# antoine311200/sow

Hardware: AMD Instinct MI355X
Metric: SoWLinear fwd+bwd tokens/s, llama_60m rank=50 (56-layer SoWLinear stack) (higher is better)
Workload: dtype bf16

## Files before the change

sow_amd/csrc/api.hip:

```cpp
#include "kernels.hpp"
#include <cstring>
#include <vector>
#include <cstdio>
#include <cstdlib>

namespace sow {

template <typename T, typename TO>
__global__ __launch_bounds__(256) void colsum_kernel(const T* M, int64_t ld, int64_t rows, int D, TO* out, float beta) {
  __shared__ float red[4][64];
  const int c = blockIdx.x * 64 + (threadIdx.x & 63), w = threadIdx.x >> 6;
  float s = 0.f;
  if (c < D)
    for (int64_t i = w; i < rows; i += 4) s += to_f32(M[i * ld + c]);
  red[w][threadIdx.x & 63] = s;
  __syncthreads();
  if (w == 0 && c < D) {
    float v = red[0][threadIdx.x] + red[1][threadIdx.x] + red[2][threadIdx.x] + red[3][threadIdx.x];
    if (beta != 0.f) v += beta * to_f32(out[c]);
    out[c] = from_f32<TO>(v);
  }
}
static int launch_colsum(const void* dy, int64_t T, int d_out, void* dbias, float beta, int dtype, int out_dtype,
                         hipStream_t stream) {
  const dim3 grid((d_out + 63) / 64);
  if (out_dtype != dtype && out_dtype != SOW_F32) return SOW_ERR_DTYPE;
  const bool o32 = out_dtype == SOW_F32;
  if (dtype == SOW_F32)
    hipLaunchKernelGGL((colsum_kernel<float, float>), grid, dim3(256), 0, stream, (const float*)dy, (int64_t)d_out, T, d_out, (float*)dbias, beta);
  else if (dtype == SOW_BF16 && o32)
    hipLaunchKernelGGL((colsum_kernel<bf16_t, float>), grid, dim3(256), 0, stream, (const bf16_t*)dy, (int64_t)d_out, T, d_out, (float*)dbias, beta);
  else if (dtype == SOW_BF16)
    hipLaunchKernelGGL((colsum_kernel<bf16_t, bf16_t>), grid, dim3(256), 0, stream, (const bf16_t*)dy, (int64_t)d_out, T, d_out, (bf16_t*)dbias, beta);
  else if (dtype == SOW_F16 && o32)
    hipLaunchKernelGGL((colsum_kernel<f16_t, float>), grid, dim3(256), 0, stream, (const f16_t*)dy, (int64_t)d_out, T, d_out, (float*)dbias, beta);
  else if (dtype == SOW_F16)
    hipLaunchKernelGGL((colsum_kernel<f16_t, f16_t>), grid, dim3(256), 0, stream, (const f16_t*)dy, (int64_t)d_out, T, d_out, (f16_t*)dbias, beta);
  else
    return SOW_ERR_DTYPE;
  SOW_CHECK_LAUNCH();
  return SOW_OK;
}
}

namespace sow {
static const char* const kSwitchNames[SW_COUNT] = {"FORCE_CHAIN_V1", "NO_SHORT_SPLIT", "NO_FUSED_H", "FORCE_GEMM_V1", "TN_NARROW",
                                                   "NO_GEMM3S",      "GEMM3S",         "GEMM3",      "NO_GROUPED",     "NO_PERSIST",     "NO_NT_STORE",    "NT_LOAD",        "NO_PAIR_FLUSH",  "F32_EXACT",
                                                   "NO_PARK16",      "TN_NO_NT_LOAD",  "NO_TN_ROWS",     "GEMM4",          "NO_GEMM4H",      "NO_CHAIN3F",     "NO_TN_F32Q",     "NO_SPLITK",
                                                   "NO_WIDE_CHAIN",  "NO_SHARED_X",    "NO_RAGGED",      "NO_RAGGED_GEMM", "NO_BLOCKED_QR",
                                                   "NO_SKINNY"};
static std::atomic<int> g_switch[SW_COUNT];
static std::once_flag g_switch_once;
static void switches_from_env() {
  for (int i = 0; i < SW_COUNT; ++i) {
    char name[64];
    snprintf(name, sizeof name, "SOW_AMD_%s", kSwitchNames[i]);
    const char* v = getenv(name);
    const bool tri = i == SW_GEMM3S || i == SW_GEMM3 || i == SW_GEMM4;
    g_switch[i].store(!v ? -1 : (tri ? (v[0] != '0') : 1), std::memory_order_relaxed);
  }
}
int sw(int which) {
  std::call_once(g_switch_once, switches_from_env);
  return g_switch[which].load(std::memory_order_relaxed);
}
}

using namespace sow;

static inline size_t al256(size_t v) { return (v + 255) & ~(size_t)255; }
static inline size_t esize(int dtype) { return dtype == SOW_F32 ? 4 : 2; }
static inline bool ok_dtype(int d) { return d == SOW_F32 || d == SOW_BF16 || d == SOW_F16; }
static inline bool al4p(const void* p) { return (reinterpret_cast<uintptr_t>(p) & 3) == 0; }
static inline bool al16p(const void* p) { return (reinterpret_cast<uintptr_t>(p) & 15) == 0; }
static inline int split_dtype(int d, bool* pf) {
  *pf = (d & SOW_PARAM_F32) != 0;
  const int cd = d & ~SOW_PARAM_F32;
  if (!ok_dtype(cd) || (*pf && cd == SOW_F32)) return -1;
  return cd;
}
static inline bool flagged(int d) { return (d & SOW_PARAM_F32) != 0; }

constexpr int SHORT_NTB = 128;
static inline int short_want(int ntb) { return ntb > 0 ? (256 + ntb - 1) / ntb : 1; }
static size_t short_hp_bytes(int64_t T, int d_in, int d_out, int r_live, int dtype) {
  const int ntb = ceil_div(T, 64);
  if (r_live > 64 || ntb <= 0 || ntb > SHORT_NTB) return 0;
  const int dmax = d_in > d_out ? d_in : d_out;
  int ks = short_want(ntb);
  const int nst = (dmax + 63) / 64;
  if (ks > nst) ks = nst;
  return al256((size_t)ks * (size_t)T * 64 * sizeof(float));
}
static int launch_chain_short(const ChainParams& p, int dtype, bool bwd, float* hpartial, hipStream_t stream) {
  const int ntb = ceil_div(p.M, 64);
  const bool f32 = dtype == SOW_F32;
  if (!hpartial || !p.Hsave || ntb > SHORT_NTB || !(f32 ? chain2f_supported(p, dtype) : chain2_supported(p, dtype)) ||
      sw_on(SW_FORCE_CHAIN_V1) || sw_on(SW_NO_SHORT_SPLIT))
    return SOW_ERR_UNSUPPORTED;
  const int want = short_want(ntb);
  const int nst = (p.D1 + 63) / 64, nsl = (p.D2 + 63) / 64;
  if (nst + nsl < 24) return SOW_ERR_UNSUPPORTED;
  int rc;
  int ks = want < nst ? want : nst;
  if (ks > 1) {
    ChainParams a = p;
    a.ntb = ntb, a.st_per = ceil_div(nst, ks), a.sl_per = 0, a.Hpartial = hpartial, a.Hload = nullptr;
    ks = ceil_div(nst, a.st_per);
    rc = f32 ? launch_chain2f(a, bwd, stream) : launch_chain2(a, bwd, dtype, stream);
    if (rc) return rc == SOW_ERR_ALIGN ? SOW_ERR_UNSUPPORTED : rc;
    rc = launch_h_reduce(hpartial, ks, p.Hsave, p.M, p.rb, p.scale, dtype, stream);
    if (rc) return rc;
  } else {
    ChainParams a = p;
    a.Y = nullptr, a.D2 = 0, a.bias = nullptr;
    rc = f32 ? launch_chain2f(a, bwd, stream) : launch_chain2(a, bwd, dtype, stream);
    if (rc) return rc == SOW_ERR_ALIGN ? SOW_ERR_UNSUPPORTED : rc;
  }
  if (nsl == 0) return SOW_OK;
  ChainParams b = p;
  const int kn = want < nsl ? want : nsl;
  b.ntb = ntb, b.st_per = 0, b.sl_per = ceil_div(nsl, kn), b.Hpartial = nullptr, b.Hload = p.Hsave, b.Hsave = nullptr;
  return f32 ? launch_chain2f(b, bwd, stream) : launch_chain2(b, bwd, dtype, stream);
}

static int gemm_auto(const void* A, int64_t lda, const void* B, int64_t ldb, bool transB, void* C, int64_t ldc,
                     const void* bias, int64_t M, int N, int K, float alpha, float beta, int dtype, hipStream_t stream,
                     void* ws = nullptr, size_t ws_bytes = 0) {
  if (dtype == SOW_F16) {
    const int g4 = sw(SW_GEMM4);
    const int64_t work = (int64_t)ceil_div(M, 256) * ceil_div(N, 256) * gemm4_splits(M, N, K, false, ws, ws_bytes);
    if (!sw_on(SW_FORCE_GEMM_V1) && (g4 > 0 || (g4 < 0 && work >= 120)) &&
        gemm4_supported(A, lda, B, ldb, transB, nullptr, 0, nullptr, 0, C, ldc, bias, M, N, K, dtype))
      return launch_gemm4(A, lda, B, ldb, transB, nullptr, 0, nullptr, 0, 0, C, ldc, bias, M, N, K, alpha, beta, stream, ws,
                          ws_bytes, dtype);
    return launch_gemm(A, lda, false, B, ldb, transB, C, ldc, bias, M, N, K, alpha, beta, dtype, stream);
  }
  if (gemm2_supported(A, lda, B, ldb, transB, nullptr, 0, nullptr, 0, C, ldc, bias, M, N, K, dtype))
    return launch_gemm2(A, lda, B, ldb, transB, nullptr, 0, nullptr, 0, 0, C, ldc, bias, M, N, K, alpha, beta, stream, ws, ws_bytes);
  return launch_gemm(A, lda, false, B, ldb, transB, C, ldc, bias, M, N, K, alpha, beta, dtype, stream);
}

extern "C" {

int sow_version(void) { return 118; }

int sow_set_switch(const char* name, int value) {
  if (!name) return SOW_ERR_NULL;
  (void)sw(0);
  for (int i = 0; i < SW_COUNT; ++i)
    if (!strcmp(name, kSwitchNames[i])) {
      g_switch[i].store(value < 0 ? -1 : (value != 0), std::memory_order_relaxed);
      return SOW_OK;
    }
  return SOW_ERR_UNSUPPORTED;
}

#ifdef SOW_STAMPS
int sow_debug_set_stamps(void* buf) {
  g_chain2_stamps = buf;
  return SOW_OK;
}
#endif

int sow_get_switch(const char* name) {
  if (!name) return SOW_ERR_NULL;
  for (int i = 0; i < SW_COUNT; ++i)
    if (!strcmp(name, kSwitchNames[i])) return sw(i);
  return SOW_ERR_UNSUPPORTED;
}

const char* sow_error_string(int code) {
  switch (code) {
    case SOW_OK: return "ok";
    case SOW_ERR_NULL: return "null pointer argument";
    case SOW_ERR_SHAPE: return "invalid shape argument";
    case SOW_ERR_DTYPE: return "unsupported dtype";
    case SOW_ERR_ALIGN: return "misaligned pointer";
    case SOW_ERR_WORKSPACE: return "workspace too small";
    case SOW_ERR_UNSUPPORTED: return "unsupported configuration";
    default: return code > 0 ? hipGetErrorString((hipError_t)code) : "unknown error";
  }
}

size_t sow_h_save_elems(int64_t T, int r_live) { return (size_t)T * (size_t)(r_live <= 64 ? 64 : r_live); }

static bool rag_layer(int r_live, int r_acc, int acc_kind, int d_in, int d_out, int dtype) {
  return r_live > 64 && ragged_shape_ok(r_live, d_in, d_out, dtype) &&
         (acc_kind == SOW_ACC_NONE || acc_kind == SOW_ACC_DENSE ||
          (acc_kind == SOW_ACC_LOWRANK && ragged_shape_ok(r_acc, d_in, d_out, dtype)));
}

static int rag_dense_product(const void* A, int64_t lda, const void* B, int64_t ldb, bool transB, void* C, int64_t ldc, int64_t M,
                             int N, int K, int dtype, hipStream_t stream) {
  if (!sw_on(SW_NO_RAGGED_GEMM) && gemm_rag_supported(A, lda, B, ldb, transB, C, ldc, M, N, K, dtype))
    return launch_gemm_rag(A, lda, B, ldb, transB, C, ldc, M, N, K, dtype, stream);
  return gemm_auto(A, lda, B, ldb, transB, C, ldc, nullptr, M, N, K, 1.f, 0.f, dtype, stream);
}

struct WsPlan {
  size_t off_dh, off_t, off_apad, off_hp, off_p0, off_p1, off_planes, planes_bytes, off_sk, sk_bytes, off_wide, wide_bytes,
      off_pw, pw_bytes, total;
  int ns, slab_len;
  int ns_cap;
};
constexpr int64_t C3F_MIN_T = 8192;
static WsPlan plan_ws(int64_t T, int d_in, int d_out, int r_live, int r_acc, int acc_kind, int dtype) {
  WsPlan w{};
  const size_t es = esize(dtype);
  size_t off = 0;
  w.off_dh = off;
  off += al256((size_t)T * (size_t)(r_live <= 64 ? 64 : r_live) * es);
  w.off_t = off;
  if (acc_kind == SOW_ACC_LOWRANK && r_acc > 64) off += al256((size_t)T * r_acc * es);
  w.off_apad = off;
  if (acc_kind == SOW_ACC_DENSE && r_live <= 64) off += al256((size_t)d_in * 64 * es);
  w.off_hp = off;
  off += short_hp_bytes(T, d_in, d_out, r_live, dtype);
  if (r_live <= 64) {
    const int cg_in = (d_in + 63) / 64, cg_out = (d_out + 63) / 64;
    const int quads = (dtype == SOW_F32 && tn_f32q_shape_ok(T, d_in, d_out)) ? (cg_in + 3) / 4 + (cg_out + 3) / 4 : 0;
    w.ns = tn_pick_slabs(T, cg_in + cg_out, (cg_in + 1) / 2 + (cg_out + 1) / 2, quads, dtype, &w.slab_len);
    w.ns_cap = w.ns;
    if (dtype == SOW_BF16 && T >= 1024) {
      const int by_len = (int)(T / 512 < TNR_MAX_SLABS ? T / 512 : TNR_MAX_SLABS);
      if (by_len > w.ns_cap) w.ns_cap = by_len;
    }
    w.off_p0 = off;
    off += al256(tn_partial_bytes(w.ns_cap, d_in));
    w.off_p1 = off;
    off += al256(tn_partial_bytes(w.ns_cap, d_out));
  }
  w.off_planes = off;
  w.planes_bytes = 0;
  if (dtype == SOW_F32 && T >= C3F_MIN_T && (r_live <= 64 || (acc_kind == SOW_ACC_LOWRANK && r_acc <= 64))) {
    w.planes_bytes = chain3f_plane_bytes(d_in, d_out);
    off += al256(w.planes_bytes);
  }
  w.off_sk = off;
  w.sk_bytes = 0;
  if (dtype == SOW_BF16 && acc_kind == SOW_ACC_DENSE) {
    const size_t f = gemm4_splitk_bytes(T, d_out, d_in, true), b = gemm4_splitk_bytes(T, d_in, d_out, true);
    w.sk_bytes = f > b ? f : b;
    off += al256(w.sk_bytes);
  }
  w.off_wide = off;
  w.wide_bytes = 0;
  {
    int rw = chain_wide_shape_ok(r_live, d_in, d_out, dtype) ? r_live : 0;
    if (acc_kind == SOW_ACC_LOWRANK && chain_wide_shape_ok(r_acc, d_in, d_out, dtype) && r_acc > rw) rw = r_acc;
    if (rag_layer(r_live, r_acc, acc_kind, d_in, d_out, dtype)) rw = acc_kind == SOW_ACC_LOWRANK && r_acc > r_live ? r_acc : r_live;
    if (rw) {
      w.wide_bytes = chain_wide_pack_bytes(rw, d_in, d_out);
      off += al256(w.wide_bytes);
    }
  }
  w.off_pw = off;
  w.pw_bytes = 0;
  if (tnw_shape_ok(r_live, d_in, d_out, dtype) || rag_layer(r_live, r_acc, acc_kind, d_in, d_out, dtype)) {
    w.pw_bytes = tnw_partial_bytes(T, d_in, d_out, r_live);
    off += al256(w.pw_bytes);
  }
  w.total = off;
  return w;
}

static char* ws_base(void* workspace) {
  uintptr_t a = reinterpret_cast<uintptr_t>(workspace);
  return reinterpret_cast<char*>((a + 255) & ~(uintptr_t)255);
}
static void set_planes(ChainParams& p, char* ws, const WsPlan& w, size_t workspace_bytes) {
  if (ws && w.planes_bytes && workspace_bytes >= w.total) p.planes = ws + w.off_planes, p.planes_bytes = w.planes_bytes;
}

static inline size_t pack_elems_bytes(int64_t n) { return al256((size_t)n * 2); }
static size_t pack_bytes(int d_in, int d_out, int r_live, int r_acc, int acc_kind) {
  size_t b = pack_elems_bytes((int64_t)d_in * r_live) + pack_elems_bytes((int64_t)r_live * d_out) + pack_elems_bytes(d_out);
  if (acc_kind == SOW_ACC_DENSE) b += pack_elems_bytes((int64_t)d_in * d_out);
  if (acc_kind == SOW_ACC_LOWRANK) b += pack_elems_bytes((int64_t)d_in * r_acc) + pack_elems_bytes((int64_t)r_acc * d_out);
  return b;
}
static int pack_layer(sow_layer_args& L, int cd, bool fwd, std::vector<PackItem>& items) {
  const int r_acc = L.acc_kind == SOW_ACC_LOWRANK ? L.r_acc : 0;
  const WsPlan w = plan_ws(L.T, L.d_in, L.d_out, L.r_live, r_acc, L.acc_kind, cd);
  const size_t pack = pack_bytes(L.d_in, L.d_out, L.r_live, r_acc, L.acc_kind);
  const bool no_scratch = fwd && sow_forward_workspace_bytes(L.T, L.d_in, L.d_out, L.r_live, r_acc, L.acc_kind, cd) == 0;
  const size_t off = (no_scratch && L.workspace_bytes < w.total + pack + 255) ? 0 : w.total;
  if (!L.workspace) return SOW_ERR_NULL;
  if (L.workspace_bytes < off + pack + 255) return SOW_ERR_WORKSPACE;
  char* dst = ws_base(L.workspace) + off;
  if (no_scratch) L.workspace = nullptr, L.workspace_bytes = 0;
  auto put = [&](const void*& src, int64_t n) {
    if (!src) return;
    items.push_back(PackItem{(const float*)src, dst, n});
    src = dst;
    dst += pack_elems_bytes(n);
  };
  put(L.A, (int64_t)L.d_in * L.r_live);
  put(L.B, (int64_t)L.r_live * L.d_out);
  put(L.bias, L.d_out);
  if (L.acc_kind == SOW_ACC_DENSE) put(L.acc_down, (int64_t)L.d_in * L.d_out);
  if (L.acc_kind == SOW_ACC_LOWRANK) {
    put(L.acc_down, (int64_t)L.d_in * r_acc);
    put(L.acc_up, (int64_t)r_acc * L.d_out);
  }
  return SOW_OK;
}
static sow_layer_args single_layer(const void* A, const void* B, const void* acc_down, const void* acc_up, const void* bias,
                                   int64_t T, int d_in, int d_out, int r_live, int r_acc, int acc_kind, void* workspace,
                                   size_t workspace_bytes) {
  sow_layer_args L{};
  L.A = A, L.B = B, L.acc_down = acc_down, L.acc_up = acc_up, L.bias = bias;
  L.T = T, L.d_in = d_in, L.d_out = d_out, L.r_live = r_live, L.r_acc = r_acc, L.acc_kind = acc_kind;
  L.workspace = workspace, L.workspace_bytes = workspace_bytes;
  return L;
}

static int wide_chain(const void* X, void* Y, const void* F1, int64_t ldf1, const void* F2, int64_t ldf2, void* Hsave,
                      const void* bias, int64_t T, int D1, int D2, int r, float hscale, float yscale, float beta, bool bwd,
                      int dtype, char* ws, const WsPlan& w, size_t workspace_bytes, hipStream_t stream, bool rag = false) {
  const bool ragged = D1 % 8 != 0 || D2 % 8 != 0;
  if ((ragged ? !rag : sw_on(SW_NO_WIDE_CHAIN)) || !ws || !w.wide_bytes || workspace_bytes < w.total + 255 ||
      chain_wide_pack_bytes(r, D1, D2) > w.wide_bytes)
    return SOW_ERR_UNSUPPORTED;
  WideArgs a{};
  a.X = X, a.Y = Y, a.F1 = F1, a.F2 = F2, a.ldf1 = ldf1, a.ldf2 = ldf2, a.Hsave = Hsave, a.bias = bias;
  a.M = T, a.D1 = D1, a.D2 = D2, a.r = r, a.hscale = hscale, a.yscale = yscale, a.beta = beta, a.bwd = bwd ? 1 : 0;
  a.pack = ws + w.off_wide, a.pack_bytes = w.wide_bytes;
  return launch_chain_wide(a, dtype, stream);
}

static ReduceParams make_reduce_params(const WsPlan& w, char* ws, void* dA, void* dB, void* dbias_ones, int d_in, int d_out,
                                       int r_live, float grad_beta) {
  ReduceParams rp{};
  rp.njobs = 2, rp.ns = w.ns;
  rp.job[0] = ReduceJob{(const float*)(ws + w.off_p0), dA, nullptr, (int64_t)r_live, d_in, (d_in + 63) / 64 * 64, r_live, 0, -1,
                        1.f, grad_beta};
  rp.job[1] = ReduceJob{(const float*)(ws + w.off_p1), dB, dbias_ones, (int64_t)d_out, d_out, (d_out + 63) / 64 * 64, r_live, 1,
                        dbias_ones ? 63 : -1, 1.f , grad_beta};
  rp.blocks0 = (d_in + 3) / 4;
  return rp;
}

size_t sow_reduce_desc_bytes(void) { return sizeof(ReduceParams); }

int sow_backward_reduce_desc(void* dA, void* dB, void* dbias, int64_t T, int d_in, int d_out, int r_live, int r_acc,
                             int acc_kind, float grad_beta, int dtype, void* workspace, size_t workspace_bytes, void* desc_out,
                             int* blocks_out) {
  bool pf;
  dtype = split_dtype(dtype, &pf);
  if (dtype < 0) return SOW_ERR_DTYPE;
  if (T <= 0 || d_in <= 0 || d_out <= 0 || r_live <= 0) return SOW_ERR_SHAPE;
  if (!dA || !dB || !workspace || !desc_out || !blocks_out) return SOW_ERR_NULL;
  if (r_live > 64) {
    memset(desc_out, 0, sizeof(ReduceParams));
    *blocks_out = 0;
    return SOW_OK;
  }
  if (dbias && r_live > 63) return SOW_ERR_UNSUPPORTED;
  if (acc_kind != SOW_ACC_LOWRANK) r_acc = 0;
  const WsPlan w = plan_ws(T, d_in, d_out, r_live, r_acc, acc_kind, dtype);
  if (workspace_bytes < w.total + 255) return SOW_ERR_WORKSPACE;
  const ReduceParams rp = make_reduce_params(w, ws_base(workspace), dA, dB, dbias, d_in, d_out, r_live, grad_beta);
  memcpy(desc_out, &rp, sizeof(rp));
  *blocks_out = (d_in + 3) / 4 + (d_out + 3) / 4;
  return SOW_OK;
}

int sow_reduce_batch(const void* descs, const int* starts, int n, int total_blocks, int dtype, void* stream) {
  bool pf;
  const int cd = split_dtype(dtype, &pf);
  if (cd < 0) return SOW_ERR_DTYPE;
  if (pf) dtype = SOW_F32;
  if (n < 0 || total_blocks < 0) return SOW_ERR_SHAPE;
  if (n == 0) return SOW_OK;
  if (!descs || !starts) return SOW_ERR_NULL;
  return launch_tn_reduce_batch((const ReduceParams*)descs, starts, n, total_blocks, dtype, (hipStream_t)stream);
}

size_t sow_forward_workspace_bytes(int64_t T, int d_in, int d_out, int r_live, int r_acc, int acc_kind, int dtype) {
  bool pf;
  dtype = split_dtype(dtype, &pf);
  if (T < 0 || d_in <= 0 || d_out <= 0 || r_live <= 0 || dtype < 0) return 0;
  if (pf) {
    const size_t own = sow_forward_workspace_bytes(T, d_in, d_out, r_live, r_acc, acc_kind, dtype);
    const size_t pack = pack_bytes(d_in, d_out, r_live, acc_kind == SOW_ACC_LOWRANK ? r_acc : 0, acc_kind);
    return own ? own + pack : pack + 256;
  }
  const bool wide_acc = acc_kind == SOW_ACC_LOWRANK && r_acc > 64;
  const WsPlan w = plan_ws(T, d_in, d_out, r_live, r_acc, acc_kind, dtype);
  if (!wide_acc && r_live <= 64 && short_hp_bytes(T, d_in, d_out, r_live, dtype) == 0 && w.planes_bytes == 0 && w.sk_bytes == 0)
    return 0;
  return w.total + 256;
}

size_t sow_workspace_bytes(int64_t T, int d_in, int d_out, int r_live, int r_acc, int acc_kind, int dtype) {
  bool pf;
  dtype = split_dtype(dtype, &pf);
  if (T < 0 || d_in <= 0 || d_out <= 0 || r_live <= 0 || dtype < 0) return 0;
  const size_t pack = pf ? pack_bytes(d_in, d_out, r_live, acc_kind == SOW_ACC_LOWRANK ? r_acc : 0, acc_kind) : 0;
  return plan_ws(T, d_in, d_out, r_live, r_acc, acc_kind, dtype).total + pack + 256;
}


static int forward_impl(const void* x, const void* A, const void* B, const void* acc_down, const void* acc_up, const void* bias,
                        void* y, void* h_save, int64_t T, int d_in, int d_out, int r_live, int r_acc, int acc_kind, float scale,
                        int dtype, void* workspace, size_t workspace_bytes, void* stream_) {
  hipStream_t stream = (hipStream_t)stream_;
  if (!ok_dtype(dtype)) return SOW_ERR_DTYPE;
  if (T < 0 || d_in <= 0 || d_out <= 0 || r_live <= 0) return SOW_ERR_SHAPE;
  if (T == 0) return SOW_OK;
  if (!x || !A || !B || !y) return SOW_ERR_NULL;
  if (acc_kind != SOW_ACC_NONE && !acc_down) return SOW_ERR_NULL;
  if (acc_kind == SOW_ACC_LOWRANK && (!acc_up || r_acc <= 0)) return SOW_ERR_SHAPE;
  if (acc_kind != SOW_ACC_LOWRANK) r_acc = 0;
  const WsPlan w = plan_ws(T, d_in, d_out, r_live, r_acc, acc_kind, dtype);
  char* ws = workspace ? ws_base(workspace) : nullptr;
  float beta = 0.f;
  int rc;
  if (rag_layer(r_live, r_acc, acc_kind, d_in, d_out, dtype) && !sw_on(SW_NO_RAGGED) && ws && workspace_bytes >= w.total + 255 &&
      al16p(x) && al16p(y) && (!bias || al16p(bias)) && (!h_save || al4p(h_save))) {
    if (acc_kind == SOW_ACC_LOWRANK) {
      rc = wide_chain(x, y, acc_down, r_acc, acc_up, d_out, nullptr, nullptr, T, d_in, d_out, r_acc, 1.f, 1.f, 0.f, false, dtype,
                      ws, w, workspace_bytes, stream, true);
      if (rc) return rc;
      beta = 1.f;
    } else if (acc_kind == SOW_ACC_DENSE) {
      rc = rag_dense_product(x, d_in, acc_down, d_out, false, y, d_out, T, d_out, d_in, dtype, stream);
      if (rc) return rc;
      beta = 1.f;
    }
    return wide_chain(x, y, A, r_live, B, d_out, h_save, bias, T, d_in, d_out, r_live, 1.f, scale, beta, false, dtype, ws, w,
                      workspace_bytes, stream, true);
  }
  if (acc_kind == SOW_ACC_DENSE) {
    if (r_live <= 64 && h_save) {
      if (gemm4h_supported(x, d_in, acc_down, d_out, false, A, r_live, B, d_out, y, d_out, bias, h_save, T, d_out, d_in, r_live,
                           dtype))
        return launch_gemm4h(x, d_in, acc_down, d_out, false, A, r_live, B, d_out, y, d_out, bias, h_save, T, d_out, d_in,
                             r_live, scale, dtype, stream);
      if (gemm2h_supported(x, d_in, acc_down, d_out, false, A, r_live, B, d_out, y, d_out, bias, h_save, T, d_out, d_in,
                           r_live, dtype))
        return launch_gemm2h(x, d_in, acc_down, d_out, false, A, r_live, B, d_out, y, d_out, bias, h_save, T, d_out, d_in,
                             r_live, scale, stream);
      ChainParams ph{};
      ph.X = x, ph.Y = nullptr, ph.Hsave = h_save, ph.bias = nullptr;
      ph.M = T, ph.ldx = d_in, ph.ldy = d_out, ph.D1 = d_in, ph.D2 = 0;
      ph.F1b = A, ph.ldf1b = r_live, ph.F2b = B, ph.ldf2b = d_out, ph.rb = r_live;
      ph.scale = scale, ph.beta = 0.f;
      set_planes(ph, ws, w, workspace_bytes);
      if (chain2_supported(ph, dtype) &&
          gemm2_supported(x, d_in, acc_down, d_out, false, h_save, 64, B, d_out, y, d_out, bias, T, d_out, d_in, dtype)) {
        rc = SOW_ERR_UNSUPPORTED;
        if (ws && workspace_bytes >= w.total) rc = launch_chain_short(ph, dtype, false, (float*)(ws + w.off_hp), stream);
        if (rc == SOW_ERR_UNSUPPORTED) rc = launch_chain2(ph, false, dtype, stream);
        if (rc) return rc;
        const bool sk = ws && w.sk_bytes && workspace_bytes >= w.total;
        return launch_gemm2(x, d_in, acc_down, d_out, false, h_save, 64, B, d_out, r_live, y, d_out, bias, T, d_out, d_in,
                            1.f, 0.f, stream, sk ? ws + w.off_sk : nullptr, sk ? w.sk_bytes : 0);
      }
    }
    rc = gemm_auto(x, d_in, acc_down, d_out, false, y, d_out, nullptr, T, d_out, d_in, 1.f, 0.f, dtype, stream);
    if (rc) return rc;
    beta = 1.f;
  } else if (acc_kind == SOW_ACC_LOWRANK) {
    if (r_acc <= 64) {
      ChainParams p{};
      p.X = x, p.Y = y, p.Hsave = nullptr, p.bias = nullptr;
      p.M = T, p.ldx = d_in, p.ldy = d_out, p.D1 = d_in, p.D2 = d_out;
      p.F1b = acc_down, p.ldf1b = r_acc, p.F2b = acc_up, p.ldf2b = d_out, p.rb = r_acc;
      p.scale = 1.f, p.beta = 0.f;
      set_planes(p, ws, w, workspace_bytes);
      rc = launch_chain(p, dtype, false, stream);
      if (rc) return rc;
      beta = 1.f;
    } else {
      if (!ws || workspace_bytes < w.total) return SOW_ERR_WORKSPACE;
      rc = wide_chain(x, y, acc_down, r_acc, acc_up, d_out, nullptr, nullptr, T, d_in, d_out, r_acc, 1.f, 1.f, 0.f, false, dtype,
                      ws, w, workspace_bytes, stream);
      if (rc == SOW_ERR_UNSUPPORTED) {
        void* t = ws + w.off_t;
        rc = launch_gemm(x, d_in, false, acc_down, r_acc, false, t, r_acc, nullptr, T, r_acc, d_in, 1.f, 0.f, dtype, stream);
        if (rc) return rc;
        rc = launch_gemm(t, r_acc, false, acc_up, d_out, false, y, d_out, nullptr, T, d_out, r_acc, 1.f, 0.f, dtype, stream);
      }
      if (rc) return rc;
      beta = 1.f;
    }
  }
  if (r_live <= 64) {
    ChainParams p{};
    p.X = x, p.Y = y, p.Hsave = h_save, p.bias = bias;
    p.M = T, p.ldx = d_in, p.ldy = d_out, p.D1 = d_in, p.D2 = d_out;
    p.F1b = A, p.ldf1b = r_live, p.F2b = B, p.ldf2b = d_out, p.rb = r_live;
    p.scale = scale, p.beta = beta;
    set_planes(p, ws, w, workspace_bytes);
    if (ws && workspace_bytes >= w.total) {
      rc = launch_chain_short(p, dtype, false, (float*)(ws + w.off_hp), stream);
      if (rc != SOW_ERR_UNSUPPORTED) return rc;
    }
    return launch_chain(p, dtype, false, stream);
  }
  const bool ws_ok = ws && workspace_bytes >= w.total + 255;
  rc = wide_chain(x, y, A, r_live, B, d_out, h_save, bias, T, d_in, d_out, r_live, 1.f, scale, beta, false, dtype, ws, w,
                  workspace_bytes, stream);
  if (rc != SOW_ERR_UNSUPPORTED) return rc;
  void* h = h_save;
  if (!h) {
    if (!ws_ok) return SOW_ERR_WORKSPACE;
    h = ws + w.off_dh;
  }
  rc = launch_gemm(x, d_in, false, A, r_live, false, h, r_live, nullptr, T, r_live, d_in, 1.f, 0.f, dtype, stream);
  if (rc) return rc;
  return launch_gemm(h, r_live, false, B, d_out, false, y, d_out, bias, T, d_out, r_live, scale, beta, dtype, stream);
}

int sow_forward(const void* x, const void* A, const void* B, const void* acc_down, const void* acc_up, const void* bias,
                void* y, void* h_save, int64_t T, int d_in, int d_out, int r_live, int r_acc, int acc_kind, float scale,
                int dtype, void* workspace, size_t workspace_bytes, void* stream) {
  bool pf;
  const int cd = split_dtype(dtype, &pf);
  if (cd < 0) return SOW_ERR_DTYPE;
  if (!pf)
    return forward_impl(x, A, B, acc_down, acc_up, bias, y, h_save, T, d_in, d_out, r_live, r_acc, acc_kind, scale, dtype,
                        workspace, workspace_bytes, stream);
  if (T < 0 || d_in <= 0 || d_out <= 0 || r_live <= 0) return SOW_ERR_SHAPE;
  if (T == 0) return SOW_OK;
  if (!x || !A || !B || !y) return SOW_ERR_NULL;
  if (acc_kind != SOW_ACC_NONE && !acc_down) return SOW_ERR_NULL;
  if (acc_kind == SOW_ACC_LOWRANK && (!acc_up || r_acc <= 0)) return SOW_ERR_SHAPE;
  if (acc_kind != SOW_ACC_LOWRANK) r_acc = 0, acc_up = nullptr;
  if (acc_kind == SOW_ACC_NONE) acc_down = nullptr;
  sow_layer_args L = single_layer(A, B, acc_down, acc_up, bias, T, d_in, d_out, r_live, r_acc, acc_kind, workspace, workspace_bytes);
  std::vector<PackItem> items;
  int rc = pack_layer(L, cd, true, items);
  if (rc) return rc;
  if ((rc = launch_pack_params(items.data(), (int)items.size(), cd, (hipStream_t)stream))) return rc;
  return forward_impl(x, L.A, L.B, L.acc_down, L.acc_up, L.bias, y, h_save, T, d_in, d_out, r_live, r_acc, acc_kind, scale, cd,
                      L.workspace, L.workspace_bytes, stream);
}

static int backward_impl(const void* dy, const void* x, const void* h_save, const void* A, const void* B, const void* acc_down,
                         const void* acc_up, void* dx, void* dA, void* dB, void* dbias, int64_t T, int d_in, int d_out,
                         int r_live, int r_acc, int acc_kind, float scale, float grad_beta, int dtype, int gdt, void* workspace,
                         size_t workspace_bytes, int phases, void* stream_) {
  hipStream_t stream = (hipStream_t)stream_;
  bool do_data = (phases & SOW_BWD_DATA) != 0;
  const bool do_partial = (phases & (SOW_BWD_WEIGHTS | SOW_BWD_WEIGHTS_PARTIAL)) != 0;
  const bool do_reduce = (phases & (SOW_BWD_WEIGHTS | SOW_BWD_WEIGHTS_REDUCE)) != 0;
  const bool do_weights = do_partial || do_reduce;
  if (!do_data && !do_weights) return SOW_ERR_SHAPE;
  if (!ok_dtype(dtype)) return SOW_ERR_DTYPE;
  if (T < 0 || d_in <= 0 || d_out <= 0 || r_live <= 0) return SOW_ERR_SHAPE;
  if (T == 0) {
    if (!dA || !dB) return SOW_ERR_NULL;
    if (grad_beta == 0.f) {
      void* ptrs[3] = {dA, dB, dbias};
      int64_t bytes[3] = {(int64_t)d_in * r_live * (int64_t)esize(gdt), (int64_t)r_live * d_out * (int64_t)esize(gdt),
                          dbias ? (int64_t)d_out * (int64_t)esize(gdt) : 0};
      return launch_multi_zero(ptrs, bytes, 3, stream);
    }
    return SOW_OK;
  }
  if (!dy || !x || !h_save || !A || !B || !dx || !dA || !dB || !workspace) return SOW_ERR_NULL;
  if (acc_kind != SOW_ACC_NONE && !acc_down) return SOW_ERR_NULL;
  if (acc_kind == SOW_ACC_LOWRANK && (!acc_up || r_acc <= 0)) return SOW_ERR_SHAPE;
  if (acc_kind != SOW_ACC_LOWRANK) r_acc = 0;
  const WsPlan w = plan_ws(T, d_in, d_out, r_live, r_acc, acc_kind, dtype);
  if (workspace_bytes < w.total + 255) return SOW_ERR_WORKSPACE;
  char* ws = ws_base(workspace);
  void* dh = ws + w.off_dh;
  float beta = 0.f;
  int rc;
  bool data_done = false;
  const bool rag_w = rag_layer(r_live, r_acc, acc_kind, d_in, d_out, dtype) && !sw_on(SW_NO_RAGGED);
  if (rag_w && do_data && al16p(dy) && al16p(dx)) {
    if (acc_kind == SOW_ACC_LOWRANK) {
      rc = wide_chain(dy, dx, acc_up, d_out, acc_down, r_acc, nullptr, nullptr, T, d_out, d_in, r_acc, 1.f, 1.f, 0.f, true, dtype,
                      ws, w, workspace_bytes, stream, true);
      if (rc) return rc;
      beta = 1.f;
    } else if (acc_kind == SOW_ACC_DENSE) {
      rc = rag_dense_product(dy, d_out, acc_down, d_out, true, dx, d_in, T, d_in, d_out, dtype, stream);
      if (rc) return rc;
      beta = 1.f;
    }
    rc = wide_chain(dy, dx, B, d_out, A, r_live, dh, nullptr, T, d_out, d_in, r_live, scale, 1.f, beta, true, dtype, ws, w,
                    workspace_bytes, stream, true);
    if (rc) return rc;
    do_data = false;
  }
  if (!do_data) {
  } else if (acc_kind == SOW_ACC_DENSE) {
    if (r_live <= 64) {
      ChainParams pd{};
      pd.X = dy, pd.Y = nullptr, pd.Hsave = dh, pd.bias = nullptr;
      pd.M = T, pd.ldx = d_out, pd.ldy = d_in, pd.D1 = d_out, pd.D2 = 0;
      pd.F1b = B, pd.ldf1b = d_out, pd.F2b = A, pd.ldf2b = r_live, pd.rb = r_live;
      pd.scale = scale, pd.beta = 0.f;
      set_planes(pd, ws, w, workspace_bytes);
      void* apad = ws + w.off_apad;
      if (gemm4h_supported(dy, d_out, acc_down, d_out, true, B, d_out, A, r_live, dx, d_in, nullptr, dh, T, d_in, d_out, r_live,
                           dtype)) {
        rc = launch_gemm4h(dy, d_out, acc_down, d_out, true, B, d_out, A, r_live, dx, d_in, nullptr, dh, T, d_in, d_out, r_live,
                           scale, dtype, stream);
        if (rc) return rc;
        data_done = true;
      } else if (gemm2h_supported(dy, d_out, acc_down, d_out, true, B, d_out, A, r_live, dx, d_in, nullptr, dh, T, d_in, d_out,
                           r_live, dtype)) {
        rc = launch_gemm2h(dy, d_out, acc_down, d_out, true, B, d_out, A, r_live, dx, d_in, nullptr, dh, T, d_in, d_out,
                           r_live, scale, stream);
        if (rc) return rc;
        data_done = true;
      } else if (chain2_supported(pd, dtype) &&
          gemm2_supported(dy, d_out, acc_down, d_out, true, dh, 64, apad, 64, dx, d_in, nullptr, T, d_in, d_out, dtype)) {
        const bool pad_fused = (int64_t)ceil_div(T, 64) * 64 >= d_in;
        if (pad_fused) pd.pad_src = A, pd.pad_dst = apad, pd.pad_rows = d_in, pd.pad_r = r_live;
        rc = SOW_ERR_UNSUPPORTED;
        if (short_hp_bytes(T, d_in, d_out, r_live, dtype)) rc = launch_chain_short(pd, dtype, true, (float*)(ws + w.off_hp), stream);
        if (rc == SOW_ERR_UNSUPPORTED) rc = launch_chain2(pd, true, dtype, stream);
        if (rc) return rc;
        if (!pad_fused) {
          rc = launch_pad64(A, apad, d_in, r_live, stream);
          if (rc) return rc;
        }
        rc = launch_gemm2(dy, d_out, acc_down, d_out, true, dh, 64, apad, 64, 64, dx, d_in, nullptr, T, d_in, d_out, 1.f, 0.f,
                          stream, w.sk_bytes ? ws + w.off_sk : nullptr, w.sk_bytes);
        if (rc) return rc;
        data_done = true;
      }
    }
    if (!data_done) rc = gemm_auto(dy, d_out, acc_down, d_out, true, dx, d_in, nullptr, T, d_in, d_out, 1.f, 0.f, dtype, stream);
    if (rc) return rc;
    beta = 1.f;
  } else if (acc_kind == SOW_ACC_LOWRANK) {
    if (r_acc <= 64) {
      ChainParams p{};
      p.X = dy, p.Y = dx, p.Hsave = nullptr, p.bias = nullptr;
      p.M = T, p.ldx = d_out, p.ldy = d_in, p.D1 = d_out, p.D2 = d_in;
      p.F1b = acc_up, p.ldf1b = d_out, p.F2b = acc_down, p.ldf2b = r_acc, p.rb = r_acc;
      p.scale = 1.f, p.beta = 0.f;
      set_planes(p, ws, w, workspace_bytes);
      rc = launch_chain(p, dtype, true, stream);
      if (rc) return rc;
      beta = 1.f;
    } else {
      rc = wide_chain(dy, dx, acc_up, d_out, acc_down, r_acc, nullptr, nullptr, T, d_out, d_in, r_acc, 1.f, 1.f, 0.f, true, dtype,
                      ws, w, workspace_bytes, stream);
      if (rc == SOW_ERR_UNSUPPORTED) {
        void* t = ws + w.off_t;
        rc = launch_gemm(dy, d_out, false, acc_up, d_out, true, t, r_acc, nullptr, T, r_acc, d_out, 1.f, 0.f, dtype, stream);
        if (rc) return rc;
        rc = launch_gemm(t, r_acc, false, acc_down, r_acc, true, dx, d_in, nullptr, T, d_in, r_acc, 1.f, 0.f, dtype, stream);
      }
      if (rc) return rc;
      beta = 1.f;
    }
  }
  if (r_live <= 64) {
    ChainParams p{};
    p.X = dy, p.Y = dx, p.Hsave = dh, p.bias = nullptr;
    p.M = T, p.ldx = d_out, p.ldy = d_in, p.D1 = d_out, p.D2 = d_in;
    p.F1b = B, p.ldf1b = d_out, p.F2b = A, p.ldf2b = r_live, p.rb = r_live;
    p.scale = scale, p.beta = beta;
    set_planes(p, ws, w, workspace_bytes);
    if (do_data && !data_done) {
      rc = launch_chain_short(p, dtype, true, short_hp_bytes(T, d_in, d_out, r_live, dtype) ? (float*)(ws + w.off_hp) : nullptr, stream);
      if (rc == SOW_ERR_UNSUPPORTED) rc = launch_chain(p, dtype, true, stream);
      if (rc) return rc;
    }
    if (!do_weights) return SOW_OK;
    const bool ones_ok = dbias && r_live <= 63;
    TnParams tp{};
    tp.njobs = 2, tp.T = T, tp.ns = w.ns, tp.slab_len = w.slab_len;
    auto vec_ok = [&](const void* ptr, int D) {
      if (dtype == SOW_F32) return (D % 4 == 0 && al16p(ptr)) ? 1 : 0;
      return (D % 2 == 0 && al4p(ptr)) ? 1 : 0;
    };
    tp.job[0] = TnJob{x, dh, (float*)(ws + w.off_p0), (int64_t)d_in, d_in, -1, (d_in + 63) / 64, vec_ok(x, d_in), 1};
    tp.job[1] = TnJob{dy, h_save, (float*)(ws + w.off_p1), (int64_t)d_out, d_out, ones_ok ? 63 : -1, (d_out + 63) / 64,
                      vec_ok(dy, d_out), 1};
    if (do_partial) {
      rc = launch_tn(tp, dtype, stream);
      if (rc) return rc;
    }
    if (!do_reduce) return SOW_OK;
    const ReduceParams rp = make_reduce_params(w, ws, dA, dB, ones_ok ? dbias : nullptr, d_in, d_out, r_live, grad_beta);
    rc = launch_tn_reduce(rp, gdt, stream);
    if (rc) return rc;
    if (dbias && !ones_ok) {
      rc = launch_colsum(dy, T, d_out, dbias, grad_beta, dtype, gdt, stream);
      if (rc) return rc;
    }
    return SOW_OK;
  }
  if (do_data) {
    rc = wide_chain(dy, dx, B, d_out, A, r_live, dh, nullptr, T, d_out, d_in, r_live, scale, 1.f, beta, true, dtype, ws, w,
                    workspace_bytes, stream);
    if (rc == SOW_ERR_UNSUPPORTED) {
      rc = launch_gemm(dy, d_out, false, B, d_out, true, dh, r_live, nullptr, T, r_live, d_out, scale, 0.f, dtype, stream);
      if (rc) return rc;
      rc = launch_gemm(dh, r_live, false, A, r_live, true, dx, d_in, nullptr, T, d_in, r_live, 1.f, beta, dtype, stream);
    }
    if (rc) return rc;
  }
  if (!do_partial) return SOW_OK;
  if (w.pw_bytes && (rag_w || (!sw_on(SW_NO_WIDE_CHAIN) && tnw_shape_ok(r_live, d_in, d_out, dtype)))) {
    rc = launch_tn_wide(x, dh, dy, h_save, dA, dB, dbias, T, d_in, d_out, r_live, scale, grad_beta, dtype, gdt, ws + w.off_pw,
                        w.pw_bytes, stream);
    if (rc != SOW_ERR_UNSUPPORTED) return rc;
  }
  rc = launch_gemm_out(x, d_in, true, dh, r_live, false, dA, r_live, nullptr, d_in, r_live, (int)T, 1.f, grad_beta, dtype, gdt,
                       stream);
  if (rc) return rc;
  rc = launch_gemm_out(h_save, r_live, true, dy, d_out, false, dB, d_out, nullptr, r_live, d_out, (int)T, scale, grad_beta, dtype,
                       gdt, stream);
  if (rc) return rc;
  if (dbias) {
    rc = launch_colsum(dy, T, d_out, dbias, grad_beta, dtype, gdt, stream);
    if (rc) return rc;
  }
  return SOW_OK;
}

int sow_backward_ex(const void* dy, const void* x, const void* h_save, const void* A, const void* B, const void* acc_down,
                    const void* acc_up, void* dx, void* dA, void* dB, void* dbias, int64_t T, int d_in, int d_out,
                    int r_live, int r_acc, int acc_kind, float scale, float grad_beta, int dtype, void* workspace,
                    size_t workspace_bytes, int phases, void* stream) {
  bool pf;
  const int cd = split_dtype(dtype, &pf);
  if (!pf)
    return backward_impl(dy, x, h_save, A, B, acc_down, acc_up, dx, dA, dB, dbias, T, d_in, d_out, r_live, r_acc, acc_kind, scale,
                         grad_beta, dtype, dtype, workspace, workspace_bytes, phases, stream);
  if (cd < 0) return SOW_ERR_DTYPE;
  if ((phases & SOW_BWD_DATA) && T > 0) {
    if (d_in <= 0 || d_out <= 0 || r_live <= 0) return SOW_ERR_SHAPE;
    if (!dy || !x || !h_save || !A || !B || !dx || !dA || !dB || !workspace) return SOW_ERR_NULL;
    if (acc_kind != SOW_ACC_NONE && !acc_down) return SOW_ERR_NULL;
    if (acc_kind == SOW_ACC_LOWRANK && (!acc_up || r_acc <= 0)) return SOW_ERR_SHAPE;
    if (acc_kind != SOW_ACC_LOWRANK) r_acc = 0, acc_up = nullptr;
    if (acc_kind == SOW_ACC_NONE) acc_down = nullptr;
    sow_layer_args L = single_layer(A, B, acc_down, acc_up, nullptr, T, d_in, d_out, r_live, r_acc, acc_kind, workspace,
                                    workspace_bytes);
    std::vector<PackItem> items;
    int rc = pack_layer(L, cd, false, items);
    if (rc) return rc;
    if ((rc = launch_pack_params(items.data(), (int)items.size(), cd, (hipStream_t)stream))) return rc;
    A = L.A, B = L.B, acc_down = L.acc_down, acc_up = L.acc_up;
  }
  return backward_impl(dy, x, h_save, A, B, acc_down, acc_up, dx, dA, dB, dbias, T, d_in, d_out, r_live, r_acc, acc_kind, scale,
                       grad_beta, cd, SOW_F32, workspace, workspace_bytes, phases, stream);
}

int sow_backward(const void* dy, const void* x, const void* h_save, const void* A, const void* B, const void* acc_down,
                 const void* acc_up, void* dx, void* dA, void* dB, void* dbias, int64_t T, int d_in, int d_out,
                 int r_live, int r_acc, int acc_kind, float scale, float grad_beta, int dtype, void* workspace,
                 size_t workspace_bytes, void* stream) {
  return sow_backward_ex(dy, x, h_save, A, B, acc_down, acc_up, dx, dA, dB, dbias, T, d_in, d_out, r_live, r_acc, acc_kind,
                         scale, grad_beta, dtype, workspace, workspace_bytes, SOW_BWD_DATA | SOW_BWD_WEIGHTS, stream);
}

static bool group_chain_params(const sow_layer_args& L, bool bwd, int dtype, const WsPlan& w, ChainParams* out) {
  if ((dtype != SOW_BF16 && dtype != SOW_F16) || L.acc_kind != SOW_ACC_NONE || L.r_live > 64 || sw_on(SW_NO_GROUPED) || sw_on(SW_FORCE_CHAIN_V1))
    return false;
  if (ceil_div(L.T, 64) <= SHORT_NTB) return false;
  ChainParams p{};
  if (!bwd) {
    p.X = L.x, p.Y = L.y, p.Hsave = L.h_save, p.bias = L.bias;
    p.M = L.T, p.ldx = L.d_in, p.ldy = L.d_out, p.D1 = L.d_in, p.D2 = L.d_out;
    p.F1b = L.A, p.ldf1b = L.r_live, p.F2b = L.B, p.ldf2b = L.d_out, p.rb = L.r_live;
  } else {
    p.X = L.dy, p.Y = L.dx, p.Hsave = ws_base(L.workspace) + w.off_dh, p.bias = nullptr;
    p.M = L.T, p.ldx = L.d_out, p.ldy = L.d_in, p.D1 = L.d_out, p.D2 = L.d_in;
    p.F1b = L.B, p.ldf1b = L.d_out, p.F2b = L.A, p.ldf2b = L.r_live, p.rb = L.r_live;
  }
  p.scale = L.scale, p.beta = 0.f;
  if (!chain2_supported(p, dtype)) return false;
  const void* Bp = bwd ? p.F1b : p.F2b;
  const int64_t ldB = bwd ? p.ldf1b : p.ldf2b;
  const void* Ap = bwd ? p.F2b : p.F1b;
  if ((reinterpret_cast<uintptr_t>(Bp) & 15) || ldB % 8 || (reinterpret_cast<uintptr_t>(Ap) & 3)) return false;
  *out = p;
  return true;
}

static bool group_rows_plan(const sow_layer_args* layers, int n, int dtype, int* ns, int* slab_len) {
  if (dtype != SOW_BF16 || n < 1 || n > TN_MAXG) return false;
  int64_t T[TNR_MAXI];
  int D[TNR_MAXI], cap[TNR_MAXI];
  for (int i = 0; i < n; ++i) {
    const sow_layer_args& L = layers[i];
    if (L.T <= 0 || L.r_live > 64 || (L.dbias && L.r_live > 63)) return false;
    const WsPlan w = plan_ws(L.T, L.d_in, L.d_out, L.r_live, L.acc_kind == SOW_ACC_LOWRANK ? L.r_acc : 0, L.acc_kind, dtype);
    if (L.workspace_bytes < w.total + 255) return false;
    if (L.d_in % 8 || L.d_out % 8 || !al16p(L.x) || !al16p(L.dy) || !al16p(L.h_save)) return false;
    T[2 * i] = T[2 * i + 1] = L.T;
    D[2 * i] = L.d_in, D[2 * i + 1] = L.d_out;
    cap[2 * i] = cap[2 * i + 1] = w.ns_cap;
  }
  return tn_rows_plan(T, D, cap, 2 * n, ns, slab_len);
}

static int check_layer(const sow_layer_args& L, bool bwd) {
  if (L.T < 0 || L.d_in <= 0 || L.d_out <= 0 || L.r_live <= 0) return SOW_ERR_SHAPE;
  if (L.T == 0) return SOW_OK;
  if (!L.x || !L.A || !L.B) return SOW_ERR_NULL;
  if (!bwd && !L.y) return SOW_ERR_NULL;
  if (bwd && (!L.dy || !L.h_save || !L.dx || !L.dA || !L.dB || !L.workspace)) return SOW_ERR_NULL;
  if (L.acc_kind != SOW_ACC_NONE && !L.acc_down) return SOW_ERR_NULL;
  return SOW_OK;
}

static int pack_group(const sow_layer_args* layers, int n, int cd, bool bwd, std::vector<sow_layer_args>& out, void* stream) {
  out.assign(layers, layers + n);
  std::vector<PackItem> items;
  int rc;
  for (sow_layer_args& L : out) {
    if ((rc = check_layer(L, bwd))) return rc;
    if (L.T == 0) continue;
    if (L.acc_kind == SOW_ACC_LOWRANK && (!L.acc_up || L.r_acc <= 0)) return SOW_ERR_SHAPE;
    if (L.acc_kind != SOW_ACC_LOWRANK) L.acc_up = nullptr;
    if (L.acc_kind == SOW_ACC_NONE) L.acc_down = nullptr;
    if (bwd) L.bias = nullptr;
    if ((rc = pack_layer(L, cd, !bwd, items))) return rc;
  }
  return launch_pack_params(items.data(), (int)items.size(), cd, (hipStream_t)stream);
}

static int forward_group_impl(const sow_layer_args* layers, int n, int dtype, void* stream_) {
  hipStream_t stream = (hipStream_t)stream_;
  if (!ok_dtype(dtype)) return SOW_ERR_DTYPE;
  if (n < 0) return SOW_ERR_SHAPE;
  if (n == 0) return SOW_OK;
  if (!layers) return SOW_ERR_NULL;
  ChainParams batch[C2_MAXG];
  Gemm2hArgs gbatch[4];
  int nb = 0, ng = 0, rc;
  for (int i = 0; i < n; ++i) {
    const sow_layer_args& L = layers[i];
    if ((rc = check_layer(L, false))) return rc;
    if (L.T == 0) continue;
    const WsPlan w{};
    if (group_chain_params(L, false, dtype, w, &batch[nb])) {
      if (++nb == C2_MAXG) {
        if ((rc = launch_chain2_group(batch, nb, false, dtype, stream))) return rc;
        nb = 0;
      }
      continue;
    }
    if (L.acc_kind == SOW_ACC_DENSE && L.r_live <= 64 && L.h_save &&
        gemm4h_supported(L.x, L.d_in, L.acc_down, L.d_out, false, L.A, L.r_live, L.B, L.d_out, L.y, L.d_out, L.bias, L.h_save, L.T,
                         L.d_out, L.d_in, L.r_live, dtype)) {
      if ((rc = launch_gemm4h(L.x, L.d_in, L.acc_down, L.d_out, false, L.A, L.r_live, L.B, L.d_out, L.y, L.d_out, L.bias, L.h_save,
                              L.T, L.d_out, L.d_in, L.r_live, L.scale, dtype, stream)))
        return rc;
      continue;
    }
    if (L.acc_kind == SOW_ACC_DENSE && L.r_live <= 64 && L.h_save && !sw_on(SW_NO_GROUPED) &&
        gemm2h_supported(L.x, L.d_in, L.acc_down, L.d_out, false, L.A, L.r_live, L.B, L.d_out, L.y, L.d_out, L.bias, L.h_save, L.T,
                         L.d_out, L.d_in, L.r_live, dtype)) {
      gbatch[ng] = Gemm2hArgs{L.x, L.acc_down, L.A, L.B, L.y, L.bias, L.h_save, L.T, L.d_in, L.d_out, L.r_live, L.d_out, L.d_out,
                              L.d_out, L.d_in, L.r_live, L.scale};
      if (++ng == 4) {
        if ((rc = launch_gemm2h_group(gbatch, ng, false, stream))) return rc;
        ng = 0;
      }
      continue;
    }
    rc = sow_forward(L.x, L.A, L.B, L.acc_down, L.acc_up, L.bias, L.y, L.h_save, L.T, L.d_in, L.d_out, L.r_live, L.r_acc,
                     L.acc_kind, L.scale, dtype, L.workspace, L.workspace_bytes, stream_);
    if (rc) return rc;
  }
  if (ng && (rc = launch_gemm2h_group(gbatch, ng, false, stream))) return rc;
  return nb ? launch_chain2_group(batch, nb, false, dtype, stream) : SOW_OK;
}

int sow_forward_group(const sow_layer_args* layers, int n, int dtype, void* stream) {
  bool pf;
  const int cd = split_dtype(dtype, &pf);
  if (cd < 0) return SOW_ERR_DTYPE;
  if (!pf || n <= 0 || !layers) return forward_group_impl(layers, n, cd, stream);
  std::vector<sow_layer_args> packed;
  const int rc = pack_group(layers, n, cd, false, packed, stream);
  return rc ? rc : forward_group_impl(packed.data(), n, cd, stream);
}

static bool skinny_shape_ok(int64_t T, int d_in, int d_out, int r_live, int acc_kind, int dtype) {
  return (dtype == SOW_BF16 || dtype == SOW_F16) && T >= 1 && T <= 32 && d_in > 0 && d_out > 0 && r_live >= 1 && r_live <= 64 &&
         (acc_kind == SOW_ACC_DENSE || acc_kind == SOW_ACC_NONE) && d_in % 8 == 0 && d_out % 8 == 0;
}
struct SkWs {
  size_t off_py, off_ph, total;
};
static SkWs skinny_ws(int64_t T, int d_in, int d_out, int acc_kind) {
  int S, KS, ncr;
  skinny_plan(d_in, d_out, acc_kind, &S, &KS, &ncr);
  SkWs w;
  w.off_py = 0;
  w.off_ph = acc_kind == SOW_ACC_DENSE ? al256(skinny_py_bytes(T, d_out, S)) : 0;
  w.total = 256 + w.off_ph + al256(skinny_ph_bytes(T, S));
  return w;
}

size_t sow_forward_skinny_workspace_bytes(int64_t T, int d_in, int d_out, int r_live, int acc_kind, int dtype) {
  if (!skinny_shape_ok(T, d_in, d_out, r_live, acc_kind, dtype)) return 0;
  return skinny_ws(T, d_in, d_out, acc_kind).total;
}

int sow_forward_skinny(const sow_layer_args* layers, int n, int dtype, void* stream) {
  bool pf;
  const int cd = split_dtype(dtype, &pf);
  if (cd < 0 || cd == SOW_F32) return SOW_ERR_DTYPE;
  if (pf || sw_on(SW_NO_SKINNY)) return SOW_ERR_UNSUPPORTED;
  if (n < 0) return SOW_ERR_SHAPE;
  if (n == 0) return SOW_OK;
  if (!layers) return SOW_ERR_NULL;
  if (n > SK_MAXL) return SOW_ERR_UNSUPPORTED;
  SkLayer sk[SK_MAXL];
  int m = 0;
  for (int i = 0; i < n; ++i) {
    const sow_layer_args& L = layers[i];
    if (L.T < 0 || L.d_in <= 0 || L.d_out <= 0 || L.r_live <= 0) return SOW_ERR_SHAPE;
    if (L.acc_kind != SOW_ACC_NONE && L.acc_kind != SOW_ACC_LOWRANK && L.acc_kind != SOW_ACC_DENSE) return SOW_ERR_SHAPE;
    if (L.T == 0) continue;
    if (!skinny_shape_ok(L.T, L.d_in, L.d_out, L.r_live, L.acc_kind, cd)) return SOW_ERR_UNSUPPORTED;
    const bool dense = L.acc_kind == SOW_ACC_DENSE;
    if (!L.x || !L.A || !L.B || !L.y || (dense && !L.acc_down)) return SOW_ERR_NULL;
    if (!al16p(L.x) || !al16p(L.y) || !al16p(L.A) || !al16p(L.B) || !al16p(L.bias) || (dense && !al16p(L.acc_down)))
      return SOW_ERR_UNSUPPORTED;
    const SkWs w = skinny_ws(L.T, L.d_in, L.d_out, L.acc_kind);
    if (!L.workspace || L.workspace_bytes < w.total) return SOW_ERR_WORKSPACE;
    char* ws = ws_base(L.workspace);
    SkLayer& K = sk[m++];
    K = SkLayer{};
    K.x = L.x, K.W = dense ? L.acc_down : nullptr, K.A = L.A, K.B = L.B, K.bias = L.bias, K.y = L.y;
    K.Py = dense ? (float*)(ws + w.off_py) : nullptr, K.Ph = (float*)(ws + w.off_ph);
    K.T = (int)L.T, K.d_in = L.d_in, K.d_out = L.d_out, K.r = L.r_live, K.scale = L.scale;
  }
  return launch_skinny_fwd(sk, m, cd, (hipStream_t)stream);
}

static int backward_group_impl(const sow_layer_args* layers, int n, int dtype, int gdt, int phases, void* stream_) {
  hipStream_t stream = (hipStream_t)stream_;
  const bool do_data = (phases & SOW_BWD_DATA) != 0;
  const bool do_partial = (phases & (SOW_BWD_WEIGHTS | SOW_BWD_WEIGHTS_PARTIAL)) != 0;
  const bool do_reduce = (phases & (SOW_BWD_WEIGHTS | SOW_BWD_WEIGHTS_REDUCE)) != 0;
  if (!do_data && !do_partial && !do_reduce) return SOW_ERR_SHAPE;
  if (!ok_dtype(dtype)) return SOW_ERR_DTYPE;
  if (n < 0) return SOW_ERR_SHAPE;
  if (n == 0) return SOW_OK;
  if (!layers) return SOW_ERR_NULL;
  int rc;
  for (int i = 0; i < n; ++i)
    if ((rc = check_layer(layers[i], true))) return rc;
  auto single = [&](const sow_layer_args& L, int ph) {
    return backward_impl(L.dy, L.x, L.h_save, L.A, L.B, L.acc_down, L.acc_up, L.dx, L.dA, L.dB, L.dbias, L.T, L.d_in, L.d_out,
                         L.r_live, L.r_acc, L.acc_kind, L.scale, L.grad_beta, dtype, gdt, L.workspace, L.workspace_bytes, ph,
                         stream_);
  };
  auto plan = [&](const sow_layer_args& L) {
    return plan_ws(L.T, L.d_in, L.d_out, L.r_live, L.acc_kind == SOW_ACC_LOWRANK ? L.r_acc : 0, L.acc_kind, dtype);
  };
  if (do_data) {
    ChainParams batch[C2_MAXG];
    Gemm2hArgs gbatch[4];
    int nb = 0, ng = 0;
    for (int i = 0; i < n; ++i) {
      const sow_layer_args& L = layers[i];
      if (L.T == 0) {
        if ((rc = single(L, SOW_BWD_DATA | (phases & ~SOW_BWD_DATA)))) return rc;
        continue;
      }
      const WsPlan w = plan(L);
      if (L.workspace_bytes < w.total + 255) return SOW_ERR_WORKSPACE;
      void* dh = ws_base(L.workspace) + w.off_dh;
      if (group_chain_params(L, true, dtype, w, &batch[nb])) {
        if (++nb == C2_MAXG) {
          if ((rc = launch_chain2_group(batch, nb, true, dtype, stream))) return rc;
          nb = 0;
        }
      } else if (L.acc_kind == SOW_ACC_DENSE && L.r_live <= 64 &&
                 gemm4h_supported(L.dy, L.d_out, L.acc_down, L.d_out, true, L.B, L.d_out, L.A, L.r_live, L.dx, L.d_in, nullptr, dh,
                                  L.T, L.d_in, L.d_out, L.r_live, dtype)) {
        if ((rc = launch_gemm4h(L.dy, L.d_out, L.acc_down, L.d_out, true, L.B, L.d_out, L.A, L.r_live, L.dx, L.d_in, nullptr, dh,
                                L.T, L.d_in, L.d_out, L.r_live, L.scale, dtype, stream)))
          return rc;
      } else if (L.acc_kind == SOW_ACC_DENSE && L.r_live <= 64 && !sw_on(SW_NO_GROUPED) &&
                 gemm2h_supported(L.dy, L.d_out, L.acc_down, L.d_out, true, L.B, L.d_out, L.A, L.r_live, L.dx, L.d_in, nullptr, dh,
                                  L.T, L.d_in, L.d_out, L.r_live, dtype)) {
        gbatch[ng] = Gemm2hArgs{L.dy, L.acc_down, L.B, L.A, L.dx, nullptr, dh, L.T, L.d_out, L.d_out, L.d_out, L.r_live, L.d_in,
                                L.d_in, L.d_out, L.r_live, L.scale};
        if (++ng == 4) {
          if ((rc = launch_gemm2h_group(gbatch, ng, true, stream))) return rc;
          ng = 0;
        }
      } else if ((rc = single(L, SOW_BWD_DATA)))
        return rc;
    }
    if (ng && (rc = launch_gemm2h_group(gbatch, ng, true, stream))) return rc;
    if (nb && (rc = launch_chain2_group(batch, nb, true, dtype, stream))) return rc;
  }
  int rns[TNR_MAXI], rslab[TNR_MAXI];
  const bool rows = (do_partial || do_reduce) && ((phases & SOW_BWD_GROUP_SLABS) || (do_partial && do_reduce)) &&
                    group_rows_plan(layers, n, dtype, rns, rslab);
  if (do_partial && rows) {
    TnRowsItem items[TNR_MAXI];
    for (int i = 0; i < n; ++i) {
      const sow_layer_args& L = layers[i];
      const WsPlan w = plan(L);
      char* ws = ws_base(L.workspace);
      items[2 * i] = TnRowsItem{L.x, ws + w.off_dh, (float*)(ws + w.off_p0), (int64_t)L.d_in, L.T, L.d_in, 0, 0, 0, 0, rns[2 * i],
                                rslab[2 * i], 0};
      items[2 * i + 1] = TnRowsItem{L.dy, L.h_save, (float*)(ws + w.off_p1), (int64_t)L.d_out, L.T, L.d_out, 0, 0, 0, 0,
                                    rns[2 * i + 1], rslab[2 * i + 1], 0};
    }
    if ((rc = launch_tn_rows(items, 2 * n, stream))) return rc;
  } else if (do_partial) {
    TnParams batch[TN_MAXG];
    int nb = 0;
    for (int i = 0; i < n; ++i) {
      const sow_layer_args& L = layers[i];
      if (L.T == 0) {
        if (!do_data && (rc = single(L, phases))) return rc;
        continue;
      }
      const WsPlan w = plan(L);
      if (L.workspace_bytes < w.total + 255) return SOW_ERR_WORKSPACE;
      bool grouped = false;
      if (L.r_live <= 64 && !sw_on(SW_NO_GROUPED)) {
        char* ws = ws_base(L.workspace);
        TnParams tp{};
        tp.njobs = 2, tp.T = L.T, tp.ns = w.ns, tp.slab_len = w.slab_len;
        const bool ones_ok = L.dbias && L.r_live <= 63;
        const int vx = (L.d_in % 2 == 0 && al4p(L.x)) ? 1 : 0, vy = (L.d_out % 2 == 0 && al4p(L.dy)) ? 1 : 0;
        tp.job[0] = TnJob{L.x, ws + w.off_dh, (float*)(ws + w.off_p0), (int64_t)L.d_in, L.d_in, -1, (L.d_in + 63) / 64, vx, 1};
        tp.job[1] = TnJob{L.dy, L.h_save, (float*)(ws + w.off_p1), (int64_t)L.d_out, L.d_out, ones_ok ? 63 : -1,
                          (L.d_out + 63) / 64, vy, 1};
        if (tn_group_supported(tp, dtype)) {
          batch[nb] = tp;
          grouped = true;
          if (++nb == TN_MAXG) {
            if ((rc = launch_tn_group(batch, nb, stream))) return rc;
            nb = 0;
          }
        }
      }
      if (!grouped && (rc = single(L, SOW_BWD_WEIGHTS_PARTIAL))) return rc;
    }
    if (nb && (rc = launch_tn_group(batch, nb, stream))) return rc;
  }
  if (do_reduce && rows) {
    for (int i = 0; i < n; ++i) {
      const sow_layer_args& L = layers[i];
      ReduceParams rp = make_reduce_params(plan(L), ws_base(L.workspace), L.dA, L.dB, L.dbias, L.d_in, L.d_out, L.r_live, L.grad_beta);
      rp.job[0].ns = rns[2 * i], rp.job[1].ns = rns[2 * i + 1];
      if ((rc = launch_tn_reduce(rp, gdt, stream))) return rc;
    }
  } else if (do_reduce) {
    for (int i = 0; i < n; ++i)
      if (layers[i].T != 0 && (rc = single(layers[i], SOW_BWD_WEIGHTS_REDUCE))) return rc;
  }
  return SOW_OK;
}

int sow_backward_group(const sow_layer_args* layers, int n, int dtype, int phases, void* stream) {
  bool pf;
  const int cd = split_dtype(dtype, &pf);
  if (!pf) return backward_group_impl(layers, n, dtype, dtype, phases, stream);
  if (cd < 0) return SOW_ERR_DTYPE;
  if (n <= 0 || !layers || !(phases & SOW_BWD_DATA)) return backward_group_impl(layers, n, cd, SOW_F32, phases, stream);
  std::vector<sow_layer_args> packed;
  const int rc = pack_group(layers, n, cd, true, packed, stream);
  return rc ? rc : backward_group_impl(packed.data(), n, cd, SOW_F32, phases, stream);
}

static int shared_common(const sow_layer_args* layers, int n, bool bwd) {
  if (n <= 0) return SOW_ERR_SHAPE;
  if (!layers) return SOW_ERR_NULL;
  for (int i = 0; i < n; ++i) {
    const sow_layer_args& L = layers[i];
    if (L.x != layers[0].x || L.T != layers[0].T || L.d_in != layers[0].d_in) return SOW_ERR_SHAPE;
    if (bwd && L.dx && L.dx != layers[0].dx) return SOW_ERR_SHAPE;
  }
  return SOW_OK;
}
static void shared_fill_dx(const sow_layer_args* layers, int n, sow_layer_args* out) {
  for (int i = 0; i < n; ++i) out[i] = layers[i], out[i].dx = layers[0].dx;
}

int sow_forward_shared(const sow_layer_args* layers, int n, int dtype, void* stream) {
  if (!ok_dtype(dtype & ~SOW_PARAM_F32)) return SOW_ERR_DTYPE;
  int rc;
  if ((rc = shared_common(layers, n, false))) return rc;
  for (int i = 0; i < n; ++i)
    if ((rc = check_layer(layers[i], false))) return rc;
  if (sw_on(SW_NO_SHARED_X) || flagged(dtype) || n > C2_MAXG || layers[0].T == 0) return SOW_ERR_UNSUPPORTED;
  ChainParams ps[C2_MAXG];
  for (int i = 0; i < n; ++i)
    if (!group_chain_params(layers[i], false, dtype, WsPlan{}, &ps[i])) return SOW_ERR_UNSUPPORTED;
  return launch_chain2_shared(ps, n, false, dtype, (hipStream_t)stream);
}

int sow_backward_shared(const sow_layer_args* layers, int n, int dtype, int phases, void* stream) {
  if (!ok_dtype(dtype & ~SOW_PARAM_F32)) return SOW_ERR_DTYPE;
  int rc;
  if ((rc = shared_common(layers, n, true))) return rc;
  if (n > C2_MAXG) return SOW_ERR_UNSUPPORTED;
  if (flagged(dtype)) return SOW_ERR_UNSUPPORTED;
  sow_layer_args filled[C2_MAXG];
  shared_fill_dx(layers, n, filled);
  if (!(phases & SOW_BWD_DATA)) return sow_backward_group(filled, n, dtype, phases, stream);
  for (int i = 0; i < n; ++i)
    if ((rc = check_layer(filled[i], true))) return rc;
  if (sw_on(SW_NO_SHARED_X) || filled[0].T == 0) return SOW_ERR_UNSUPPORTED;
  ChainParams ps[C2_MAXG];
  for (int i = 0; i < n; ++i) {
    const sow_layer_args& L = filled[i];
    const WsPlan w = plan_ws(L.T, L.d_in, L.d_out, L.r_live, 0, L.acc_kind, dtype);
    if (!group_chain_params(L, true, dtype, w, &ps[i])) return SOW_ERR_UNSUPPORTED;
    if (L.workspace_bytes < w.total + 255) return SOW_ERR_WORKSPACE;
    ps[i].beta = filled[0].grad_beta;
  }
  if ((rc = launch_chain2_shared(ps, n, true, dtype, (hipStream_t)stream))) return rc;
  const int wph = phases & ~SOW_BWD_DATA;
  return (wph & (SOW_BWD_WEIGHTS | SOW_BWD_WEIGHTS_PARTIAL | SOW_BWD_WEIGHTS_REDUCE))
             ? backward_group_impl(filled, n, dtype, dtype, wph, stream)
             : SOW_OK;
}

int sow_backward_group_plan(const sow_layer_args* layers, int n, int dtype, int phases, int* slabs_out) {
  bool pf;
  dtype = split_dtype(dtype, &pf);
  if (dtype < 0) return SOW_ERR_DTYPE;
  if (n < 0) return SOW_ERR_SHAPE;
  if (n == 0) return 0;
  if (!layers) return SOW_ERR_NULL;
  int rc;
  for (int i = 0; i < n; ++i)
    if ((rc = check_layer(layers[i], true))) return rc;
  const bool do_partial = (phases & (SOW_BWD_WEIGHTS | SOW_BWD_WEIGHTS_PARTIAL)) != 0;
  const bool do_reduce = (phases & (SOW_BWD_WEIGHTS | SOW_BWD_WEIGHTS_REDUCE)) != 0;
  int rns[TNR_MAXI], rslab[TNR_MAXI];
  const bool rows = (do_partial || do_reduce) && ((phases & SOW_BWD_GROUP_SLABS) || (do_partial && do_reduce)) &&
                    group_rows_plan(layers, n, dtype, rns, rslab);
  if (slabs_out)
    for (int i = 0; i < n; ++i) {
      const sow_layer_args& L = layers[i];
      int ns = 0;
      if (L.T > 0 && L.r_live <= 64)
        ns = plan_ws(L.T, L.d_in, L.d_out, L.r_live, L.acc_kind == SOW_ACC_LOWRANK ? L.r_acc : 0, L.acc_kind, dtype).ns;
      slabs_out[2 * i] = rows ? rns[2 * i] : ns;
      slabs_out[2 * i + 1] = rows ? rns[2 * i + 1] : ns;
    }
  return rows ? 1 : 0;
}

int sow_backward_group_reduce_desc(const sow_layer_args* layers, int n, int dtype, int phases, void* descs_out, int* blocks_out) {
  bool pf;
  dtype = split_dtype(dtype, &pf);
  if (dtype < 0) return SOW_ERR_DTYPE;
  if (n < 0) return SOW_ERR_SHAPE;
  if (n == 0) return SOW_OK;
  if (!layers || !descs_out || !blocks_out) return SOW_ERR_NULL;
  int rc;
  for (int i = 0; i < n; ++i)
    if ((rc = check_layer(layers[i], true))) return rc;
  int rns[TNR_MAXI], rslab[TNR_MAXI];
  const bool rows = (phases & SOW_BWD_GROUP_SLABS) && group_rows_plan(layers, n, dtype, rns, rslab);
  for (int i = 0; i < n; ++i) {
    const sow_layer_args& L = layers[i];
    char* out = (char*)descs_out + (size_t)i * sizeof(ReduceParams);
    if ((rc = sow_backward_reduce_desc(L.dA, L.dB, L.dbias, L.T, L.d_in, L.d_out, L.r_live, L.r_acc, L.acc_kind, L.grad_beta, dtype,
                                       L.workspace, L.workspace_bytes, out, blocks_out + i)))
      return rc;
    if (rows) {
      ReduceParams rp;
      memcpy(&rp, out, sizeof rp);
      rp.job[0].ns = rns[2 * i], rp.job[1].ns = rns[2 * i + 1];
      memcpy(out, &rp, sizeof rp);
    }
  }
  return SOW_OK;
}

int sow_gemm(const void* A, int64_t lda, int trans_a, const void* B, int64_t ldb, int trans_b, void* C, int64_t ldc,
             const void* bias, int64_t M, int N, int K, float alpha, float beta, int dtype, void* stream) {
  return sow_gemm_ex(A, lda, trans_a, B, ldb, trans_b, C, ldc, bias, M, N, K, alpha, beta, dtype, nullptr, 0, stream);
}

size_t sow_gemm_workspace_bytes(int64_t M, int N, int K, int trans_a, int dtype) {
  if (trans_a || (dtype != SOW_BF16 && dtype != SOW_F16) || M <= 0 || N <= 0 || K <= 0) return 0;
  return gemm4_splitk_bytes(M, N, K, false);
}

int sow_gemm_ex(const void* A, int64_t lda, int trans_a, const void* B, int64_t ldb, int trans_b, void* C, int64_t ldc,
                const void* bias, int64_t M, int N, int K, float alpha, float beta, int dtype, void* workspace,
                size_t workspace_bytes, void* stream) {
  if (flagged(dtype)) return SOW_ERR_DTYPE;
  if (!trans_a)
    return gemm_auto(A, lda, B, ldb, trans_b != 0, C, ldc, bias, M, N, K, alpha, beta, dtype, (hipStream_t)stream, workspace,
                     workspace_bytes);
  return launch_gemm(A, lda, trans_a != 0, B, ldb, trans_b != 0, C, ldc, bias, M, N, K, alpha, beta, dtype, (hipStream_t)stream);
}

constexpr int QR_BLOCK_MIN = 64;
constexpr int QR_TAIL_K = 512;
struct QrPlan {
  int kc;
  size_t off_pt, off_qt, off_w, off_r, total;
  size_t off_t, total_thin;
};
static QrPlan plan_qr(int m, int n, int k, int in_dtype, int need_r, int out_dtype_is_f32) {
  QrPlan q{};
  q.kc = k < m ? k : m;
  if (n < q.kc) q.kc = n;
  size_t off = 0;
  q.off_pt = off;
  off += al256((size_t)q.kc * m * 4);
  q.off_qt = off;
  off += al256((size_t)k * m * 4);
  q.off_w = off;
  if (need_r && n > q.kc && in_dtype != SOW_F32) off += al256((size_t)m * (n - q.kc) * 4);
  q.off_r = off;
  if (need_r && n > q.kc && !out_dtype_is_f32) off += al256((size_t)k * (n - q.kc) * 4);
  q.total = off;
  q.off_t = off;
  if (q.kc > QR_BLOCK_MIN) off += al256(qr_blocked_t_floats(q.kc) * 4);
  q.total_thin = off;
  return q;
}

size_t sow_qr_workspace_bytes(int m, int n, int k, int in_dtype, int need_r) {
  if (m <= 0 || n <= 0 || k <= 0) return 0;
  return plan_qr(m, n, k, in_dtype, need_r, 0).total_thin + 256;
}

int sow_qr_thin(const void* W, int64_t ldw, int m, int n, int in_dtype, int k, void* Q_out, int64_t ldq, void* R_out,
                int64_t ldr, int out_dtype, void* workspace, size_t workspace_bytes, void* stream_) {
  hipStream_t stream = (hipStream_t)stream_;
  if (!ok_dtype(in_dtype) || !ok_dtype(out_dtype)) return SOW_ERR_DTYPE;
  if (m <= 0 || n <= 0 || k <= 0 || k > m) return SOW_ERR_SHAPE;
  if (!W || !Q_out || !workspace) return SOW_ERR_NULL;
  const QrPlan q = plan_qr(m, n, k, in_dtype, R_out != nullptr, out_dtype == SOW_F32);
  if (workspace_bytes < q.total_thin + 255) return SOW_ERR_WORKSPACE;
  char* ws = ws_base(workspace);
  float* Pt = (float*)(ws + q.off_pt);
  float* Qt = (float*)(ws + q.off_qt);
  int rc;
  const bool blocked = q.kc > QR_BLOCK_MIN && !sw_on(SW_NO_BLOCKED_QR);
  if (blocked)
    rc = launch_qr_blocked(W, ldw, in_dtype, m, q.kc, k, Pt, Qt, (float*)(ws + q.off_t), stream);
  else
    rc = launch_qr_panel(W, ldw, in_dtype, m, q.kc, k, Pt, Qt, stream);
  if (rc) return rc;
  rc = launch_qr_copy_out(Qt, Pt, Q_out, ldq, R_out, ldr, out_dtype, m, q.kc, k, k, stream);
  if (rc) return rc;
  if (R_out && n > q.kc) {
    const int nt = n - q.kc;
    const void* Bp;
    int64_t ldb;
    if (in_dtype == SOW_F32) {
      Bp = (const float*)W + q.kc, ldb = ldw;
    } else {
      float* wf = (float*)(ws + q.off_w);
      rc = launch_cast_copy((const char*)W + q.kc * esize(in_dtype), ldw, in_dtype, wf, nt, SOW_F32, m, nt, stream);
      if (rc) return rc;
      Bp = wf, ldb = nt;
    }
    const int kstep = blocked ? QR_TAIL_K : m;
    float* rt = out_dtype == SOW_F32 ? (float*)R_out + q.kc : (float*)(ws + q.off_r);
    const int64_t ldt = out_dtype == SOW_F32 ? ldr : nt;
    for (int k0 = 0; k0 < m; k0 += kstep) {
      const int kk = m - k0 < kstep ? m - k0 : kstep;
      rc = launch_gemm(Qt + k0, m, false, (const float*)Bp + (int64_t)k0 * ldb, ldb, false, rt, ldt, nullptr, k, nt, kk, 1.f,
                       k0 ? 1.f : 0.f, SOW_F32, stream);
      if (rc) return rc;
    }
    if (out_dtype != SOW_F32) {
      rc = launch_cast_copy(rt, nt, SOW_F32, (char*)R_out + q.kc * esize(out_dtype), ldr, out_dtype, k, nt, stream);
      if (rc) return rc;
    }
  }
  return SOW_OK;
}

int sow_accumulate_batch(const sow_accumulate_args* items, int n, int dtype, void* stream_) {
  hipStream_t stream = (hipStream_t)stream_;
  if (!ok_dtype(dtype)) return SOW_ERR_DTYPE;
  if (n < 0) return SOW_ERR_SHAPE;
  if (n == 0) return SOW_OK;
  if (!items) return SOW_ERR_NULL;
  std::vector<AccItem> its((size_t)n);
  std::vector<void*> zp;
  std::vector<int64_t> zb;
  for (int i = 0; i < n; ++i) {
    const sow_accumulate_args& a = items[i];
    if (a.d_in <= 0 || a.d_out <= 0 || a.r <= 0 || a.r > 64) return SOW_ERR_SHAPE;
    if (!a.acc || !a.A || !a.B) return SOW_ERR_NULL;
    AccItem& t = its[(size_t)i];
    t.acc = a.acc, t.A = a.A, t.B = a.B, t.draw = a.draw, t.A_new = a.A_new, t.ld_draw = a.ld_draw;
    t.d_in = a.d_in, t.d_out = a.d_out, t.r = a.r, t.r_new = a.r_new, t.scale = a.scale, t.beta = a.acc_beta;
    t.Pt = t.Qt = nullptr, t.kc = 0;
    if (a.draw) {
      if (!a.A_new || !a.workspace || a.r_new <= 0 || a.r_new > a.d_in || a.draw_cols <= 0 || a.ld_draw < a.draw_cols)
        return a.A_new && a.workspace ? SOW_ERR_SHAPE : SOW_ERR_NULL;
      const QrPlan q = plan_qr(a.d_in, a.draw_cols, a.r_new, dtype, 0, 0);
      if (a.workspace_bytes < q.total + 255) return SOW_ERR_WORKSPACE;
      char* ws = ws_base(a.workspace);
      t.kc = q.kc, t.Pt = (float*)(ws + q.off_pt), t.Qt = (float*)(ws + q.off_qt);
    }
    if (a.zero && a.zero_bytes > 0) zp.push_back(a.zero), zb.push_back(a.zero_bytes);
  }
  int rc = launch_accumulate_batch(its.data(), n, dtype, stream);
  if (rc) return rc;
  return zp.empty() ? SOW_OK : launch_multi_zero(zp.data(), zb.data(), (int)zp.size(), stream);
}

int sow_zero_state(void* const* ptrs, const int64_t* bytes, int n, void* stream) {
  if (n < 0) return SOW_ERR_SHAPE;
  if (n == 0) return SOW_OK;
  if (!ptrs || !bytes) return SOW_ERR_NULL;
  return launch_multi_zero(ptrs, bytes, n, (hipStream_t)stream);
}

int sow_adamw_flat(void* param, const void* grad, void* exp_avg, void* exp_avg_sq, int64_t n, float lr, double beta1,
                   double beta2, float eps, float weight_decay, int step, float grad_scale, int dtype, int state_dtype,
                   void* stream) {
  if (flagged(dtype) || flagged(state_dtype)) return SOW_ERR_DTYPE;
  if (step < 1) return SOW_ERR_SHAPE;
  return launch_adamw_flat(param, grad, exp_avg, exp_avg_sq, n, lr, beta1, beta2, eps, weight_decay, step, grad_scale,
                           dtype, state_dtype, (hipStream_t)stream);
}

int sow_ttadam_dense(float* param, const float* grad, float* exp_avg, float* exp_avg_sq, int64_t n, double beta1,
                     double beta2, float eps, float step_size, float lr_times_wd, int clamp_v, void* stream) {
  return launch_ttadam_dense(param, grad, exp_avg, exp_avg_sq, n, beta1, beta2, eps, step_size, lr_times_wd, clamp_v,
                             (hipStream_t)stream);
}

int sow_tt_kron_core(const float* A, const float* B, float* out, int ra0, int rb0, int ij, int ra1, int rb1,
                     void* stream) {
  return launch_tt_kron_core(A, B, out, ra0, rb0, ij, ra1, rb1, (hipStream_t)stream);
}

int sow_absmax(const float* x, int64_t n, float* out, void* stream) {
  return launch_absmax(x, n, out, (hipStream_t)stream);
}

int sow_small_inverse(const float* A, float* out, int batch, int r, void* stream) {
  return launch_small_inverse(A, out, batch, r, (hipStream_t)stream);
}

int sow_axpby(const void* x, void* y, int64_t n, float a, float b, int dtype, void* stream) {
  if (flagged(dtype)) return SOW_ERR_DTYPE;
  return launch_axpby(x, y, n, a, b, dtype, (hipStream_t)stream);
}

int sow_cast_copy(const void* src, int64_t lds, int src_dtype, void* dst, int64_t ldd, int dst_dtype, int64_t rows,
                  int cols, void* stream) {
  if (flagged(src_dtype) || flagged(dst_dtype) || !ok_dtype(src_dtype) || !ok_dtype(dst_dtype)) return SOW_ERR_DTYPE;
  if (!src || !dst) return SOW_ERR_NULL;
  return launch_cast_copy(src, lds, src_dtype, dst, ldd, dst_dtype, rows, cols, (hipStream_t)stream);
}

}
```

sow_amd/csrc/common.hpp:

```cpp
#pragma once
#include <hip/hip_runtime.h>
#include <stdint.h>

#include <atomic>
#include <mutex>

#include "../../include/sow_amd.h"

namespace sow {

typedef __bf16 bf16_t;
typedef __attribute__((ext_vector_type(8))) __bf16 bf16x8;
typedef __attribute__((ext_vector_type(4))) __bf16 bf16x4;
typedef __attribute__((ext_vector_type(2))) __bf16 bf16x2;
typedef _Float16 f16_t;
typedef __attribute__((ext_vector_type(8))) _Float16 f16x8;
typedef __attribute__((ext_vector_type(2))) _Float16 f16x2;
typedef __attribute__((ext_vector_type(16))) float f32x16;
typedef __attribute__((ext_vector_type(4))) float f32x4;
typedef __attribute__((ext_vector_type(2))) float f32x2;
typedef __attribute__((ext_vector_type(4))) uint32_t u32x4;
typedef __attribute__((ext_vector_type(2))) uint32_t u32x2;

enum : int { SOW_F32 = 0, SOW_BF16 = 1, SOW_F16 = 2 };


template <typename T> struct DT;
template <> struct DT<float> {
  static constexpr int id = SOW_F32;
  static constexpr int VE = 4;
  using v8 = float;
};
template <> struct DT<bf16_t> {
  static constexpr int id = SOW_BF16;
  static constexpr int VE = 8;
  using v8 = bf16x8;
  static constexpr uint32_t one_bits = 0x3F80u;
};
template <> struct DT<f16_t> {
  static constexpr int id = SOW_F16;
  static constexpr int VE = 8;
  using v8 = f16x8;
  static constexpr uint32_t one_bits = 0x3C00u;
};

__device__ __forceinline__ float to_f32(float v) { return v; }
__device__ __forceinline__ float to_f32(bf16_t v) { return (float)v; }
__device__ __forceinline__ float to_f32(f16_t v) { return (float)v; }
template <typename T> __device__ __forceinline__ T from_f32(float v);
template <> __device__ __forceinline__ float from_f32<float>(float v) { return v; }
template <> __device__ __forceinline__ bf16_t from_f32<bf16_t>(float v) { return (bf16_t)v; }
template <> __device__ __forceinline__ f16_t from_f32<f16_t>(float v) { return (f16_t)v; }

__device__ __forceinline__ f32x16 mfma32(bf16x8 a, bf16x8 b, f32x16 c) {
  return __builtin_amdgcn_mfma_f32_32x32x16_bf16(a, b, c, 0, 0, 0);
}
__device__ __forceinline__ f32x16 mfma32(f16x8 a, f16x8 b, f32x16 c) {
  return __builtin_amdgcn_mfma_f32_32x32x16_f16(a, b, c, 0, 0, 0);
}
__device__ __forceinline__ f32x16 mfma32(float a, float b, f32x16 c) {
  return __builtin_amdgcn_mfma_f32_32x32x2f32(a, b, c, 0, 0, 0);
}

__device__ __forceinline__ int acc_row(int reg, int lane) { return (reg & 3) + 8 * (reg >> 2) + 4 * (lane >> 5); }

template <int KT> __device__ __forceinline__ int bf16_img_chunk(int row, int c) {
  constexpr int NC = KT / 8;
  constexpr int RPB = 16 / NC;
  static_assert(NC == 4 || NC == 8 || NC == 16, "KT must be 32, 64 or 128");
  return c ^ ((row / RPB) & (NC - 1));
}
template <int KT> __device__ __forceinline__ int bf16_img_off(int row, int c) {
  return row * (KT * 2) + bf16_img_chunk<KT>(row, c) * 16;
}

__device__ __forceinline__ void transpose_8x2(const uint32_t (&d)[8], u32x4& col0, u32x4& col1) {
#pragma unroll
  for (int m = 0; m < 4; ++m) {
    uint32_t a = d[2 * m], b = d[2 * m + 1];
    col0[m] = (a & 0xffffu) | (b << 16);
    col1[m] = (a >> 16) | (b & 0xffff0000u);
  }
}

__device__ __forceinline__ uint32_t pack_bf16x2(float lo, float hi) {
  bf16x2 v;
  v[0] = (bf16_t)lo;
  v[1] = (bf16_t)hi;
  return __builtin_bit_cast(uint32_t, v);
}
__device__ __forceinline__ uint32_t pack_f16x2(float lo, float hi) {
  f16x2 v;
  v[0] = (f16_t)lo;
  v[1] = (f16_t)hi;
  return __builtin_bit_cast(uint32_t, v);
}
template <typename T> __device__ __forceinline__ uint32_t pack16x2(float lo, float hi);
template <> __device__ __forceinline__ uint32_t pack16x2<bf16_t>(float lo, float hi) { return pack_bf16x2(lo, hi); }
template <> __device__ __forceinline__ uint32_t pack16x2<f16_t>(float lo, float hi) { return pack_f16x2(lo, hi); }
template <typename T> __device__ __forceinline__ typename DT<T>::v8 as_v8(u32x4 v) {
  return __builtin_bit_cast(typename DT<T>::v8, v);
}

__device__ __forceinline__ int xcd_remap(int bid, int nwg) {
  const int q = nwg >> 3, r = nwg & 7, xcd = bid & 7, idx = bid >> 3;
  return (xcd < r ? xcd * (q + 1) : r * (q + 1) + (xcd - r) * q) + idx;
}

inline int ceil_div(int64_t a, int64_t b) { return (int)((a + b - 1) / b); }

#define SOW_SET_MAX_LDS_ONCE(bytes, ...)                                                                            \
  do {                                                                                                              \
    static std::atomic<uint64_t> done__{0};                                                                         \
    int dev__ = 0;                                                                                                  \
    (void)hipGetDevice(&dev__);                                                                                     \
    const uint64_t bit__ = 1ull << (dev__ & 63);                                                                    \
    if (!(done__.load(std::memory_order_acquire) & bit__)) {                                                        \
      (void)hipFuncSetAttribute((const void*)(__VA_ARGS__), hipFuncAttributeMaxDynamicSharedMemorySize, (bytes));    \
      done__.fetch_or(bit__, std::memory_order_release);                                                            \
    }                                                                                                               \
  } while (0)

enum Switch : int {
  SW_FORCE_CHAIN_V1 = 0,
  SW_NO_SHORT_SPLIT,
  SW_NO_FUSED_H,
  SW_FORCE_GEMM_V1,
  SW_TN_NARROW,
  SW_NO_GEMM3S,
  SW_GEMM3S,
  SW_GEMM3,
  SW_NO_GROUPED,
  SW_NO_PERSIST,
  SW_NO_NT_STORE,
  SW_NT_LOAD,
  SW_NO_PAIR_FLUSH,
  SW_F32_EXACT,
  SW_NO_PARK16,
  SW_TN_NO_NT_LOAD,
  SW_NO_TN_ROWS,
  SW_GEMM4,
  SW_NO_GEMM4H,
  SW_NO_CHAIN3F,
  SW_NO_TN_F32Q,
  SW_NO_SPLITK,
  SW_NO_WIDE_CHAIN,
  SW_NO_SHARED_X,
  SW_NO_RAGGED,
  SW_NO_RAGGED_GEMM,
  SW_NO_BLOCKED_QR,
  SW_NO_SKINNY,
  SW_COUNT
};
int sw(int which);
inline bool sw_on(int which) { return sw(which) > 0; }

#ifdef SOW_GEMM_NO_NT
#define SOW_GEMM_NT(M) false
#else
#define SOW_GEMM_NT(M) ((M) >= 8192)
#endif

#define SOW_CHECK_LAUNCH()                     \
  do {                                         \
    hipError_t e__ = hipGetLastError();        \
    if (e__ != hipSuccess) return (int)e__;    \
  } while (0)

}
```

sow_amd/csrc/gemm4.hip:

```cpp
#include "kernels.hpp"
#include "lds_dma.hpp"
#include <type_traits>

namespace sow {

constexpr int G4_BM = 256, G4_BN = 256, G4_BK = 64;
constexpr int G4_THREADS = 512;
constexpr int G4_HALF = 128 * G4_BK * 2;
constexpr int G4_BUF = 4 * G4_HALF;
constexpr int G4_LDS = 2 * G4_BUF;
constexpr int G4_OFF_A0 = 0, G4_OFF_A1 = G4_HALF, G4_OFF_B0 = 2 * G4_HALF, G4_OFF_B1 = 3 * G4_HALF;
constexpr int G4_SCR_LD = 68;
constexpr int G4_SCR = 16 * G4_SCR_LD * 4;
constexpr int G4_HIMG = G4_LDS;
constexpr int G4_LDS_H = G4_LDS + 2 * G4_HALF;
constexpr int G4_PA_BUF = 2 * G4_HALF + 8192;

struct Gemm4Params {
  const bf16_t* A;
  const bf16_t* B;
  const bf16_t* A2;
  const bf16_t* B2;
  bf16_t* C;
  const bf16_t* bias;
  int64_t M, lda, ldb, lda2, ldb2, ldc;
  int N, K, k2;
  int k2e;
  float alpha, beta;
  int nt_store;
  const bf16_t* F;
  int64_t ldf;
  bf16_t* Hout;
  int r;
  float hscale;
  int splits, kt_per;
  float* partials;
};

__device__ __forceinline__ f32x4 mfma16(u32x4 a, u32x4 b, f32x4 c) {
  return __builtin_amdgcn_mfma_f32_16x16x32_bf16(as_bf16x8(a), as_bf16x8(b), c, 0, 0, 0);
}
__device__ __forceinline__ f32x4 mfma16_f16(u32x4 a, u32x4 b, f32x4 c) {
  return __builtin_amdgcn_mfma_f32_16x16x32_f16(as_v8<f16_t>(a), as_v8<f16_t>(b), c, 0, 0, 0);
}

template <int OFF> __device__ __forceinline__ void g4_rd128(u32x4& d, uint32_t a) {
  asm volatile("ds_read_b128 %0, %1 offset:%2" : "=v"(d) : "v"(a), "n"(OFF) : "memory");
}
template <int OFF> __device__ __forceinline__ void g4_rdtr(u32x2& d, uint32_t a) {
  asm volatile("ds_read_b64_tr_b16 %0, %1 offset:%2" : "=v"(d) : "v"(a), "n"(OFF) : "memory");
}
template <int MH> __device__ __forceinline__ void g4_read_a(u32x4 (&af)[4][2], uint32_t a0, uint32_t a1) {
  g4_rd128<MH * G4_HALF + 0 * 2048>(af[0][0], a0);
  g4_rd128<MH * G4_HALF + 0 * 2048>(af[0][1], a1);
  g4_rd128<MH * G4_HALF + 1 * 2048>(af[1][0], a0);
  g4_rd128<MH * G4_HALF + 1 * 2048>(af[1][1], a1);
  g4_rd128<MH * G4_HALF + 2 * 2048>(af[2][0], a0);
  g4_rd128<MH * G4_HALF + 2 * 2048>(af[2][1], a1);
  g4_rd128<MH * G4_HALF + 3 * 2048>(af[3][0], a0);
  g4_rd128<MH * G4_HALF + 3 * 2048>(af[3][1], a1);
}
template <int NH> __device__ __forceinline__ void g4_read_b_nt(u32x4 (&bf)[2][2], uint32_t b0, uint32_t b1) {
  g4_rd128<NH * G4_HALF + 0 * 2048>(bf[0][0], b0);
  g4_rd128<NH * G4_HALF + 0 * 2048>(bf[0][1], b1);
  g4_rd128<NH * G4_HALF + 1 * 2048>(bf[1][0], b0);
  g4_rd128<NH * G4_HALF + 1 * 2048>(bf[1][1], b1);
}
template <int NH> __device__ __forceinline__ void g4_read_b_nn(u32x2 (&bl)[2][2], u32x2 (&bh)[2][2], uint32_t n0a, uint32_t n1a) {
  g4_rdtr<NH * G4_HALF + 0>(bl[0][0], n0a);
  g4_rdtr<NH * G4_HALF + 1024>(bh[0][0], n0a);
  g4_rdtr<NH * G4_HALF + 8192>(bl[0][1], n0a);
  g4_rdtr<NH * G4_HALF + 8192 + 1024>(bh[0][1], n0a);
  g4_rdtr<NH * G4_HALF + 0>(bl[1][0], n1a);
  g4_rdtr<NH * G4_HALF + 1024>(bh[1][0], n1a);
  g4_rdtr<NH * G4_HALF + 8192>(bl[1][1], n1a);
  g4_rdtr<NH * G4_HALF + 8192 + 1024>(bh[1][1], n1a);
}

enum : int { G4_A0 = 0, G4_B0 = 1, G4_B1 = 2, G4_A1 = 3 };
template <int KIND> __device__ __forceinline__ constexpr int g4_slot_off() {
  return KIND == G4_A0 ? G4_OFF_A0 : KIND == G4_A1 ? G4_OFF_A1 : KIND == G4_B0 ? G4_OFF_B0 : G4_OFF_B1;
}

#define G4_KERNEL gemm4_kernel
#define G4_REDUCE gemm4_splitk_reduce_kernel
#define G4_T bf16_t
#define G4_MFMA mfma16
#define G4_PACK pack_bf16x2
#define G4_ONE 0x3F80u
#include "gemm4_body.hpp"
#undef G4_KERNEL
#undef G4_REDUCE
#undef G4_T
#undef G4_MFMA
#undef G4_PACK
#undef G4_ONE
#define G4_KERNEL gemm4_f16_kernel
#define G4_REDUCE gemm4_f16_splitk_reduce_kernel
#define G4_T f16_t
#define G4_MFMA mfma16_f16
#define G4_PACK pack_f16x2
#define G4_ONE 0x3C00u
#include "gemm4_body.hpp"
#undef G4_KERNEL
#undef G4_REDUCE
#undef G4_T
#undef G4_MFMA
#undef G4_PACK
#undef G4_ONE

static bool g4_al16(const void* q) { return (reinterpret_cast<uintptr_t>(q) & 15) == 0; }

bool gemm4_supported(const void* A, int64_t lda, const void* B, int64_t ldb, bool nt, const void* A2, int64_t lda2,
                     const void* B2, int64_t ldb2, const void* C, int64_t ldc, const void* bias, int64_t M, int N, int K,
                     int dtype) {
  if ((dtype != SOW_BF16 && dtype != SOW_F16) || !A || !B || !C) return false;
  if (M < 1 || N < 64 || K < 64) return false;
  if (K % 8 || N % 8 || lda % 8 || ldb % 8 || ldc % 8) return false;
  if (!g4_al16(A) || !g4_al16(B) || !g4_al16(C) || (bias && !g4_al16(bias))) return false;
  if (A2 && (!B2 || lda2 % 8 || ldb2 % 8 || !g4_al16(A2) || !g4_al16(B2))) return false;
  (void)nt;
  return true;
}

static int gemm4_split_plan(int64_t M, int N, int K, bool has_ext, int* kt_per) {
  const int64_t tiles = (int64_t)ceil_div(M, G4_BM) * ceil_div(N, G4_BN);
  const int ntl = ceil_div(K, G4_BK) + (has_ext ? 1 : 0);
  *kt_per = ntl;
  if (tiles <= 0 || tiles > 128 || ntl < 96 || sw_on(SW_NO_SPLITK)) return 1;
  int s = (int)(256 / tiles);
  if (s > 4) s = 4;
  while (s > 1 && ntl / s < 8) --s;
  if (s <= 1) return 1;
  *kt_per = ceil_div(ntl, s);
  return ceil_div(ntl, *kt_per);
}
size_t gemm4_splitk_bytes(int64_t M, int N, int K, bool has_ext) {
  int kt_per;
  const int s = gemm4_split_plan(M, N, K, has_ext, &kt_per);
  if (s <= 1) return 0;
  return (size_t)s * (size_t)M * (size_t)N * sizeof(float) + 256;
}
int gemm4_splits(int64_t M, int N, int K, bool has_ext, const void* ws, size_t ws_bytes) {
  int kt_per;
  const int s = gemm4_split_plan(M, N, K, has_ext, &kt_per);
  return (s > 1 && ws && ws_bytes >= gemm4_splitk_bytes(M, N, K, has_ext)) ? s : 1;
}

int launch_gemm4(const void* A, int64_t lda, const void* B, int64_t ldb, bool nt, const void* A2, int64_t lda2,
                 const void* B2, int64_t ldb2, int k2, void* C, int64_t ldc, const void* bias, int64_t M, int N, int K,
                 float alpha, float beta, hipStream_t stream, void* ws, size_t ws_bytes, int dtype) {
  if (dtype != SOW_BF16 && dtype != SOW_F16) return SOW_ERR_DTYPE;
  const bool f16 = dtype == SOW_F16;
  Gemm4Params p;
  p.A = (const bf16_t*)A, p.B = (const bf16_t*)B, p.A2 = (const bf16_t*)A2, p.B2 = (const bf16_t*)B2;
  p.C = (bf16_t*)C, p.bias = (const bf16_t*)bias;
  p.M = M, p.lda = lda, p.ldb = ldb, p.lda2 = lda2, p.ldb2 = ldb2, p.ldc = ldc;
  p.N = N, p.K = K, p.k2 = k2 < 64 ? k2 : 64;
  p.k2e = 64;
  p.alpha = alpha, p.beta = beta;
  p.nt_store = SOW_GEMM_NT(M) ? 1 : 0;
  p.F = nullptr, p.ldf = 0, p.Hout = nullptr, p.r = 0, p.hscale = 0.f;
  p.splits = 1, p.kt_per = 0, p.partials = nullptr;
  const int64_t tiles = (int64_t)ceil_div(M, G4_BM) * ceil_div(N, G4_BN);
  if (tiles <= 0) return SOW_OK;
  if (tiles > 0x7fffffff) return SOW_ERR_SHAPE;
  int64_t grid = tiles;
  if (gemm4_splits(M, N, K, A2 != nullptr, ws, ws_bytes) > 1) {
    p.splits = gemm4_split_plan(M, N, K, A2 != nullptr, &p.kt_per);
    p.partials = (float*)(((uintptr_t)ws + 255) & ~(uintptr_t)255);
    grid = tiles * p.splits;
  }
#define G4_LAUNCH(K, LDS, ...)                                                                                   \
  do {                                                                                                           \
    SOW_SET_MAX_LDS_ONCE(LDS, K<__VA_ARGS__>);                                                                   \
    hipLaunchKernelGGL((K<__VA_ARGS__>), dim3((unsigned)grid), dim3(G4_THREADS), LDS, stream, p);               \
  } while (0)
  if (p.splits > 1 && nt) {
    if (f16) G4_LAUNCH(gemm4_f16_kernel, G4_LDS, true, false, true);
    else G4_LAUNCH(gemm4_kernel, G4_LDS, true, false, true);
  } else if (p.splits > 1) {
    if (f16) G4_LAUNCH(gemm4_f16_kernel, G4_LDS, false, false, true);
    else G4_LAUNCH(gemm4_kernel, G4_LDS, false, false, true);
  } else if (nt) {
    if (f16) G4_LAUNCH(gemm4_f16_kernel, G4_LDS, true, false);
    else G4_LAUNCH(gemm4_kernel, G4_LDS, true, false);
  } else {
    if (f16) G4_LAUNCH(gemm4_f16_kernel, G4_LDS, false, false);
    else G4_LAUNCH(gemm4_kernel, G4_LDS, false, false);
  }
  SOW_CHECK_LAUNCH();
  if (p.splits > 1) {
    const int64_t work = M * (N / 8);
    const dim3 rgrid((unsigned)((work + 255) / 256));
    if (f16)
      hipLaunchKernelGGL(gemm4_f16_splitk_reduce_kernel, rgrid, dim3(256), 0, stream, p.partials, p.splits, M, N, (f16_t*)p.C, p.ldc,
                         (const f16_t*)p.bias, p.alpha, p.beta);
    else
      hipLaunchKernelGGL(gemm4_splitk_reduce_kernel, rgrid, dim3(256), 0, stream, p.partials, p.splits, M, N, p.C, p.ldc, p.bias,
                         p.alpha, p.beta);
    SOW_CHECK_LAUNCH();
  }
  return SOW_OK;
}

bool gemm4h_supported(const void* X, int64_t ldx, const void* W, int64_t ldw, bool nt, const void* F, int64_t ldf,
                      const void* G, int64_t ldg, const void* C, int64_t ldc, const void* bias, const void* H, int64_t M,
                      int N, int K, int r, int dtype) {
  if ((dtype != SOW_BF16 && dtype != SOW_F16) || !X || !W || !F || !G || !C || !H) return false;
  if (sw_on(SW_NO_FUSED_H) || sw_on(SW_FORCE_GEMM_V1) || sw(SW_GEMM4) == 0 || sw_on(SW_NO_GEMM4H)) return false;
  if (r < 2 || r > 64 || (r & 1) || N < 64 || K < 64) return false;
  const int tiles_n = ceil_div(N, G4_BN);
  if (tiles_n > 2 || (int64_t)ceil_div(M, G4_BM) * tiles_n < 120) return false;
  if (K % 8 || N % 8 || ldx % 8 || ldw % 8 || ldc % 8) return false;
  if (!g4_al16(X) || !g4_al16(W) || !g4_al16(C) || !g4_al16(H) || (bias && !g4_al16(bias))) return false;
  auto al4 = [](const void* q) { return (reinterpret_cast<uintptr_t>(q) & 3) == 0; };
  if (nt) {
    if (ldf % 8 || !g4_al16(F) || !al4(G) || (ldg != r && ldg != 64)) return false;
  } else {
    if (ldg % 8 || !g4_al16(G) || !al4(F) || (ldf != r && ldf != 64)) return false;
  }
  return true;
}

int launch_gemm4h(const void* X, int64_t ldx, const void* W, int64_t ldw, bool nt, const void* F, int64_t ldf,
                  const void* G, int64_t ldg, void* C, int64_t ldc, const void* bias, void* H, int64_t M, int N, int K,
                  int r, float hscale, int dtype, hipStream_t stream) {
  if (dtype != SOW_BF16 && dtype != SOW_F16) return SOW_ERR_DTYPE;
  const bool f16 = dtype == SOW_F16;
  Gemm4Params p;
  p.A = (const bf16_t*)X, p.B = (const bf16_t*)W, p.A2 = nullptr, p.B2 = (const bf16_t*)G;
  p.C = (bf16_t*)C, p.bias = (const bf16_t*)bias;
  p.M = M, p.lda = ldx, p.ldb = ldw, p.lda2 = 64, p.ldb2 = ldg, p.ldc = ldc;
  p.N = N, p.K = K, p.k2 = r < 64 ? r : 64;
  p.k2e = nt ? (ldg == 64 ? 64 : r) : 64;
  p.alpha = 1.f, p.beta = 0.f;
  p.nt_store = SOW_GEMM_NT(M) ? 1 : 0;
  p.F = (const bf16_t*)F, p.ldf = ldf, p.Hout = (bf16_t*)H, p.r = r, p.hscale = hscale;
  p.splits = 1, p.kt_per = 0, p.partials = nullptr;
  const int64_t tiles = (int64_t)ceil_div(M, G4_BM) * ceil_div(N, G4_BN);
  if (tiles <= 0) return SOW_OK;
  if (tiles > 0x7fffffff) return SOW_ERR_SHAPE;
  const int64_t grid = tiles;
  if (nt) {
    if (f16) G4_LAUNCH(gemm4_f16_kernel, G4_LDS_H, true, true);
    else G4_LAUNCH(gemm4_kernel, G4_LDS_H, true, true);
  } else {
    if (f16) G4_LAUNCH(gemm4_f16_kernel, G4_LDS_H, false, true);
    else G4_LAUNCH(gemm4_kernel, G4_LDS_H, false, true);
  }
#undef G4_LAUNCH
  SOW_CHECK_LAUNCH();
  return SOW_OK;
}

}
```

sow_amd/csrc/gemm4_body.hpp:

```cpp

template <bool NT, bool HF, bool SK = false> __global__ __launch_bounds__(G4_THREADS, 2) void G4_KERNEL(const Gemm4Params p) {
  extern __shared__ __attribute__((aligned(16))) char smem[];
  const int t = threadIdx.x, lane = t & 63;
  const int w = __builtin_amdgcn_readfirstlane(t >> 6);
  const int wr = w >> 2, wc = w & 3;
  const int r16 = lane & 15, g = lane >> 4;
  const int tiles_n = (p.N + G4_BN - 1) / G4_BN;
  const int splits = SK ? p.splits : 1;
  const int ntiles = (int)gridDim.x / splits;
  const int split = splits > 1 ? (int)blockIdx.x / ntiles : 0;
  const int lid = splits > 1 ? (int)blockIdx.x % ntiles : xcd_remap(blockIdx.x, gridDim.x);
  const int64_t m0 = (int64_t)(lid / tiles_n) * G4_BM;
  const int n0 = (lid % tiles_n) * G4_BN;
  const int K = p.K, N = p.N;
  const int64_t M = p.M;
  const int nfull = K / G4_BK;
  const bool has_ext = HF || p.A2 != nullptr;
  const int NTL_all = nfull + ((K % G4_BK) ? 1 : 0) + (has_ext ? 1 : 0);
  const int kt0 = splits > 1 ? split * p.kt_per : 0;
  const int NTL = splits > 1 ? (kt0 + p.kt_per < NTL_all ? kt0 + p.kt_per : NTL_all) : NTL_all;
  const int H = 4 * NTL;
  const char* zp = zero_page_for(lane);

  const int c_pc = lane & 7;
  int c_lr[2], c_q[2];
#pragma unroll
  for (int ii = 0; ii < 2; ++ii) {
    c_lr[ii] = 16 * w + 8 * ii + (lane >> 3);
    c_q[ii] = c_pc ^ ((c_lr[ii] >> 1) & 7);
  }
  auto a_row = [&](int mh, int lr) -> int64_t {
    const int64_t gr = m0 + (lr >> 6) * 128 + mh * 64 + (lr & 63);
    return gr < M ? gr : M - 1;
  };
  auto b_col_nt = [&](int nh, int lr) -> int {
    const int gn = n0 + (lr >> 5) * 64 + nh * 32 + (lr & 31);
    return gn < N ? gn : N - 1;
  };
  const int m_kr0 = 8 * w + (lane >> 4);
  const int m_f = (((lane >> 4) & 3) | ((w & 1) << 2)) << 1;
  const int m_q = (lane & 15) ^ m_f;
  auto b_col_nn = [&](int nh) -> int {
    const int lc = 8 * m_q;
    const int gn = n0 + (lc >> 5) * 64 + nh * 32 + (lc & 31);
    return gn + 8 <= N ? gn : N - 8;
  };

  const bf16_t* pA[2][2];
  const bf16_t* pB[2][2];
#pragma unroll
  for (int hh = 0; hh < 2; ++hh)
#pragma unroll
    for (int ii = 0; ii < 2; ++ii) {
      pA[hh][ii] = p.A + a_row(hh, c_lr[ii]) * p.lda + 8 * c_q[ii];
      if constexpr (NT) pB[hh][ii] = p.B + (int64_t)b_col_nt(hh, c_lr[ii]) * p.ldb + 8 * c_q[ii];
      else pB[hh][ii] = p.B + (int64_t)(m_kr0 + 4 * ii) * p.ldb + b_col_nn(hh);
    }
  const int64_t stepB = NT ? (int64_t)G4_BK : (int64_t)G4_BK * p.ldb;
  if (kt0 > 0) {
#pragma unroll
    for (int hh = 0; hh < 2; ++hh)
#pragma unroll
      for (int ii = 0; ii < 2; ++ii) pA[hh][ii] += (int64_t)kt0 * G4_BK, pB[hh][ii] += (int64_t)kt0 * stepB;
  }

  auto issue = [&](auto kind_c, int tile) {
    constexpr int KIND = decltype(kind_c)::value;
    constexpr bool IS_A = KIND == G4_A0 || KIND == G4_A1;
    constexpr int HH = (KIND == G4_A1 || KIND == G4_B1) ? 1 : 0;
    char* dst = smem + (tile & 1) * G4_BUF + g4_slot_off<KIND>() + (2 * w) * 1024;
    if (tile < nfull) {
#pragma unroll
      for (int ii = 0; ii < 2; ++ii) {
        if constexpr (IS_A) {
          dma16(pA[HH][ii], dst + ii * 1024);
          pA[HH][ii] += G4_BK;
        } else {
          dma16(pB[HH][ii], dst + ii * 1024);
          pB[HH][ii] += stepB;
        }
      }
      return;
    }
    const bool ext = has_ext && tile == NTL_all - 1;
    const int k0 = ext ? 0 : nfull * G4_BK;
#pragma unroll
    for (int ii = 0; ii < 2; ++ii) {
      const void* src;
      if constexpr (IS_A) {
        const bf16_t* base = ext ? p.A2 : p.A;
        const int64_t ld = ext ? p.lda2 : p.lda;
        const int klim = ext ? 64 : K;
        const int kk = k0 + 8 * c_q[ii];
        src = (kk < klim && !(HF && ext)) ? (const void*)(base + a_row(HH, c_lr[ii]) * ld + kk) : (const void*)zp;
      } else if constexpr (NT) {
        const bf16_t* base = ext ? p.B2 : p.B;
        const int64_t ld = ext ? p.ldb2 : p.ldb;
        const int klim = ext ? p.k2e : K;
        const int kk = k0 + 8 * c_q[ii];
        const int64_t eoff = (int64_t)b_col_nt(HH, c_lr[ii]) * ld + kk;
        const bool ok = kk < klim && !(HF && ext && eoff + 8 > (int64_t)N * ld);
        src = ok ? (const void*)(base + eoff) : (const void*)zp;
      } else {
        const bf16_t* base = ext ? p.B2 : p.B;
        const int64_t ld = ext ? p.ldb2 : p.ldb;
        const int krows = ext ? p.k2 : K;
        const int gk = k0 + m_kr0 + 4 * ii;
        src = gk < krows ? (const void*)(base + (int64_t)gk * ld + b_col_nn(HH)) : (const void*)zp;
      }
      dma16(src, dst + ii * 1024);
    }
  };
  using KA0 = std::integral_constant<int, G4_A0>;
  using KB0 = std::integral_constant<int, G4_B0>;
  using KB1 = std::integral_constant<int, G4_B1>;
  using KA1 = std::integral_constant<int, G4_A1>;

  if constexpr (HF) {
    const int NTA = (K + G4_BK - 1) / G4_BK;
    const int f_row = 8 * w + (lane >> 3);
    const int f_pc = lane & 7;
    const int f_q = NT ? (f_pc ^ ((f_row >> 1) & 7)) : (f_pc ^ ((((lane >> 4) & 1) | ((w & 1) << 1)) << 1));
    auto issue_a = [&](int tl) {
      char* buf = smem + (tl % 3) * G4_PA_BUF;
      const int k0 = tl * G4_BK;
#pragma unroll
      for (int hh = 0; hh < 2; ++hh)
#pragma unroll
        for (int ii = 0; ii < 2; ++ii) {
          const void* src = (k0 + 8 * c_q[ii] < K) ? (const void*)pA[hh][ii] : (const void*)zp;
          dma16(src, buf + hh * G4_HALF + (2 * w + ii) * 1024);
          pA[hh][ii] += G4_BK;
        }
      const void* fs;
      if constexpr (NT) {
        const int kk = k0 + 8 * f_q;
        fs = (f_row < p.r && kk < K) ? (const void*)(p.F + (int64_t)f_row * p.ldf + kk) : (const void*)zp;
      } else {
        const int gk = k0 + f_row;
        const int64_t eoff = (int64_t)gk * p.ldf + 8 * f_q;
        const bool ok = gk < K && 8 * f_q < p.r && eoff + 8 <= (int64_t)K * p.ldf;
        fs = ok ? (const void*)(p.F + eoff) : (const void*)zp;
      }
      dma16(fs, buf + 2 * G4_HALF + w * 1024);
    };
    auto patch_f = [&](int tl) {
      if constexpr (!NT) {
        const int gk = tl * G4_BK + f_row;
        const int64_t eoff = (int64_t)gk * p.ldf + 8 * f_q;
        if (gk < K && 8 * f_q < p.r && eoff + 8 > (int64_t)K * p.ldf) {
          u32x4 v;
          bf16_t* e = (bf16_t*)&v;
#pragma unroll
          for (int j = 0; j < 8; ++j) e[j] = (8 * f_q + j < p.r) ? p.F[eoff + j] : (bf16_t)0.f;
          *(u32x4*)(smem + (tl % 3) * G4_PA_BUF + 2 * G4_HALF + w * 1024 + lane * 16) = v;
          asm volatile("s_waitcnt lgkmcnt(0)" ::: "memory");
        }
      }
    };
    const uint32_t lbase = lds_addr(smem);
    const int fsw_a = (r16 >> 1) & 7;
    const int cha = (fsw_a & 4) | (g ^ (fsw_a & 3));
    const uint32_t ar0 = lbase + (uint32_t)((wr * 64 + r16) * 128 + cha * 16);
    const uint32_t ar1 = lbase + (uint32_t)((wr * 64 + r16) * 128 + (cha ^ 4) * 16);
    uint32_t fr0, fr1;
    if constexpr (NT) {
      fr0 = lbase + (uint32_t)(2 * G4_HALF + (wc * 16 + r16) * 128 + cha * 16);
      fr1 = lbase + (uint32_t)(2 * G4_HALF + (wc * 16 + r16) * 128 + (cha ^ 4) * 16);
    } else {
      const int qq = r16 >> 2, pp = r16 & 3;
      const int ff_sw = (((qq >> 1) & 1) | ((g & 1) << 1)) << 1;
      const int chunk = wc * 2 + (pp >> 1);
      fr0 = lbase + (uint32_t)(2 * G4_HALF + (8 * g + qq) * 128 + ((chunk ^ ff_sw) * 16) + 8 * (pp & 1));
      fr1 = fr0;
    }
    f32x4 hacc[2][4];
#pragma unroll
    for (int a = 0; a < 2; ++a)
#pragma unroll
      for (int b = 0; b < 4; ++b) hacc[a][b] = (f32x4){0.f, 0.f, 0.f, 0.f};
    issue_a(0);
    if (NTA > 1) issue_a(1);
#pragma unroll 1
    for (int tl = 0; tl < NTA; ++tl) {
      wait_groups<5>(NTA - 1 - tl < 1 ? NTA - 1 - tl : 1);
      if (tl == NTA - 1) patch_f(tl);
      __builtin_amdgcn_s_barrier();
      __builtin_amdgcn_sched_barrier(0);
      if (tl + 2 < NTA) issue_a(tl + 2);
      const uint32_t bo = (uint32_t)((tl % 3) * G4_PA_BUF);
      u32x4 xa[4][2], ffr[2];
      u32x2 fl[2], fh[2];
      g4_read_a<0>(xa, ar0 + bo, ar1 + bo);
      if constexpr (NT) {
        g4_rd128<0>(ffr[0], fr0 + bo);
        g4_rd128<0>(ffr[1], fr1 + bo);
      } else {
        g4_rdtr<0>(fl[0], fr0 + bo);
        g4_rdtr<512>(fh[0], fr0 + bo);
        g4_rdtr<4096>(fl[1], fr0 + bo);
        g4_rdtr<4096 + 512>(fh[1], fr0 + bo);
      }
      asm volatile("s_waitcnt lgkmcnt(0)" ::: "memory");
      __builtin_amdgcn_sched_barrier(0);
      if constexpr (!NT) ffr[0] = join2(fl[0], fh[0]), ffr[1] = join2(fl[1], fh[1]);
#pragma unroll
      for (int ks = 0; ks < 2; ++ks)
#pragma unroll
        for (int mt = 0; mt < 4; ++mt) hacc[0][mt] = G4_MFMA(ffr[ks], xa[mt][ks], hacc[0][mt]);
      __builtin_amdgcn_sched_barrier(0);
      g4_read_a<1>(xa, ar0 + bo, ar1 + bo);
      asm volatile("s_waitcnt lgkmcnt(0)" ::: "memory");
      __builtin_amdgcn_sched_barrier(0);
#pragma unroll
      for (int ks = 0; ks < 2; ++ks)
#pragma unroll
        for (int mt = 0; mt < 4; ++mt) hacc[1][mt] = G4_MFMA(ffr[ks], xa[mt][ks], hacc[1][mt]);
      __builtin_amdgcn_sched_barrier(0);
    }
#pragma unroll
    for (int mh = 0; mh < 2; ++mh)
#pragma unroll
      for (int mt = 0; mt < 4; ++mt) {
        const int lr = wr * 64 + mt * 16 + r16;
        const int q = wc * 2 + (g >> 1);
        char* dst = smem + G4_HIMG + mh * G4_HALF + lr * 128 + ((q ^ ((lr >> 1) & 7)) * 16) + (g & 1) * 8;
        f32x4 v = hacc[mh][mt];
#pragma unroll
        for (int j = 0; j < 4; ++j) v[j] = (wc * 16 + 4 * g + j < p.r) ? v[j] * p.hscale : 0.f;
        *(u32x2*)dst = (u32x2){G4_PACK(v[0], v[1]), G4_PACK(v[2], v[3])};
      }
    asm volatile("s_waitcnt lgkmcnt(0)" ::: "memory");
    __builtin_amdgcn_s_barrier();
    __builtin_amdgcn_sched_barrier(0);
#pragma unroll
    for (int hh = 0; hh < 2; ++hh)
#pragma unroll
      for (int ii = 0; ii < 2; ++ii) pA[hh][ii] = p.A + a_row(hh, c_lr[ii]) * p.lda + 8 * c_q[ii];
  }

  const uint32_t base = lds_addr(smem);
  const int fsw = (r16 >> 1) & 7;
  const int ch0 = (fsw & 4) | (g ^ (fsw & 3));
  uint32_t a_off[2], b_off[2];
  a_off[0] = base + (uint32_t)((wr * 64 + r16) * 128 + ch0 * 16);
  a_off[1] = base + (uint32_t)((wr * 64 + r16) * 128 + (ch0 ^ 4) * 16);
  if constexpr (NT) {
    b_off[0] = base + (uint32_t)(G4_OFF_B0 + (wc * 32 + r16) * 128 + ch0 * 16);
    b_off[1] = base + (uint32_t)(G4_OFF_B0 + (wc * 32 + r16) * 128 + (ch0 ^ 4) * 16);
  } else {
    const int qq = r16 >> 2, pp = r16 & 3;
    const int f = (qq | ((g & 1) << 2)) << 1;
#pragma unroll
    for (int nt = 0; nt < 2; ++nt) {
      const int chunk = wc * 4 + nt * 2 + (pp >> 1);
      b_off[nt] = base + (uint32_t)(G4_OFF_B0 + (8 * g + qq) * 256 + ((chunk ^ f) * 16) + 8 * (pp & 1));
    }
  }

  f32x4 acc[2][4][2][2];
#pragma unroll
  for (int a = 0; a < 2; ++a)
#pragma unroll
    for (int b = 0; b < 4; ++b)
#pragma unroll
      for (int c = 0; c < 2; ++c)
#pragma unroll
        for (int d = 0; d < 2; ++d) acc[a][b][c][d] = (f32x4){0.f, 0.f, 0.f, 0.f};
  u32x4 af[4][2];
  u32x4 bf[2][2][2];
  u32x2 bl[2][2][2], bh[2][2][2];

  auto read_a = [&](auto mh_c) { g4_read_a<decltype(mh_c)::value>(af, a_off[0], a_off[1]); };
  auto read_b = [&](auto nh_c) {
    constexpr int NH = decltype(nh_c)::value;
    if constexpr (NT) g4_read_b_nt<NH>(bf[NH], b_off[0], b_off[1]);
    else g4_read_b_nn<NH>(bl[NH], bh[NH], b_off[0], b_off[1]);
  };
  using I0 = std::integral_constant<int, 0>;
  using I1 = std::integral_constant<int, 1>;

  auto phase = [&](auto ph_c, auto tail_c, int tile) {
    constexpr int PH = decltype(ph_c)::value;
    constexpr bool TAIL = decltype(tail_c)::value;
    constexpr int MH = PH >= 2 ? 1 : 0;
    constexpr int NH = (PH == 1 || PH == 2) ? 1 : 0;
    if constexpr (PH == 0) {
      read_b(I0{});
      __builtin_amdgcn_sched_barrier(0);
      read_a(I0{});
    } else if constexpr (PH == 1) {
      read_b(I1{});
    } else if constexpr (PH == 2) {
      read_a(I1{});
    }
    __builtin_amdgcn_sched_barrier(0);
    const int P = 4 * tile + PH;
    const int h = P + 6;
    if (!TAIL || h < H) {
      if constexpr (PH == 0) issue(KB1{}, h >> 2);
      else if constexpr (PH == 1) issue(KA1{}, h >> 2);
      else if constexpr (PH == 2) issue(KA0{}, h >> 2);
      else issue(KB0{}, h >> 2);
    }
    if constexpr (!TAIL) {
      asm volatile("s_waitcnt vmcnt(8)" ::: "memory");
      __builtin_amdgcn_sched_barrier(0);
    } else {
      int newer = H - 3 - P;
      newer = newer < 0 ? 0 : (newer > 4 ? 4 : newer);
      wait_groups<2>(newer);
    }
    __builtin_amdgcn_s_barrier();
    asm volatile("s_waitcnt lgkmcnt(0)" ::: "memory");
    __builtin_amdgcn_sched_barrier(0);
    __builtin_amdgcn_s_setprio(1);
#pragma unroll
    for (int ks = 0; ks < 2; ++ks)
#pragma unroll
      for (int mt = 0; mt < 4; ++mt)
#pragma unroll
        for (int nt = 0; nt < 2; ++nt) {
          u32x4 wf;
          if constexpr (NT) wf = bf[NH][nt][ks];
          else wf = join2(bl[NH][nt][ks], bh[NH][nt][ks]);
          acc[MH][mt][NH][nt] = G4_MFMA(wf, af[mt][ks], acc[MH][mt][NH][nt]);
        }
    __builtin_amdgcn_s_setprio(0);
    __builtin_amdgcn_sched_barrier(0);
    __builtin_amdgcn_s_barrier();
    __builtin_amdgcn_sched_barrier(0);
    if constexpr (PH == 3) {
      a_off[0] ^= G4_BUF, a_off[1] ^= G4_BUF, b_off[0] ^= G4_BUF, b_off[1] ^= G4_BUF;
    }
  };
  using T0 = std::integral_constant<bool, false>;
  using T1 = std::integral_constant<bool, true>;
  using P0 = std::integral_constant<int, 0>;
  using P1 = std::integral_constant<int, 1>;
  using P2 = std::integral_constant<int, 2>;
  using P3 = std::integral_constant<int, 3>;

  if (kt0 & 1) a_off[0] ^= G4_BUF, a_off[1] ^= G4_BUF, b_off[0] ^= G4_BUF, b_off[1] ^= G4_BUF;
  issue(KA0{}, kt0), issue(KB0{}, kt0), issue(KB1{}, kt0), issue(KA1{}, kt0);
  if (NTL - kt0 > 1) issue(KA0{}, kt0 + 1), issue(KB0{}, kt0 + 1);
  wait_groups<2>(NTL - kt0 > 1 ? 4 : 2);
  __builtin_amdgcn_s_barrier();
  __builtin_amdgcn_sched_barrier(0);
  if (wr == 1) __builtin_amdgcn_s_barrier();
  __builtin_amdgcn_sched_barrier(0);

  int tile = kt0;
#pragma unroll 1
  for (; tile < NTL - 2; ++tile) {
    phase(P0{}, T0{}, tile);
    phase(P1{}, T0{}, tile);
    phase(P2{}, T0{}, tile);
    phase(P3{}, T0{}, tile);
  }
#pragma unroll 1
  for (; tile < NTL - 1; ++tile) {
    phase(P0{}, T1{}, tile);
    phase(P1{}, T1{}, tile);
    phase(P2{}, T1{}, tile);
    phase(P3{}, T1{}, tile);
  }
  if (tile < NTL) {
    if constexpr (HF) {
      if (tile == NTL - 1) {
        a_off[0] = base + (uint32_t)(G4_HIMG + (wr * 64 + r16) * 128 + ch0 * 16);
        a_off[1] = base + (uint32_t)(G4_HIMG + (wr * 64 + r16) * 128 + (ch0 ^ 4) * 16);
        if constexpr (NT) {
          if (p.ldb2 != 64) {
            asm volatile("s_waitcnt vmcnt(0)" ::: "memory");
            __builtin_amdgcn_sched_barrier(0);
#pragma unroll
            for (int hh = 0; hh < 2; ++hh)
#pragma unroll
              for (int ii = 0; ii < 2; ++ii) {
                const int kk = 8 * c_q[ii];
                const int64_t eoff = (int64_t)b_col_nt(hh, c_lr[ii]) * p.ldb2 + kk;
                if (kk < p.k2e && eoff + 8 > (int64_t)N * p.ldb2) {
                  u32x4 v;
                  bf16_t* e = (bf16_t*)&v;
#pragma unroll
                  for (int j = 0; j < 8; ++j) e[j] = (kk + j < p.k2e) ? p.B2[eoff + j] : (bf16_t)0.f;
                  *(u32x4*)(smem + (tile & 1) * G4_BUF + (hh ? G4_OFF_B1 : G4_OFF_B0) + (2 * w + ii) * 1024 + lane * 16) = v;
                }
              }
            asm volatile("s_waitcnt vmcnt(0) lgkmcnt(0)" ::: "memory");
            __builtin_amdgcn_s_barrier();
            __builtin_amdgcn_s_barrier();
            __builtin_amdgcn_sched_barrier(0);
          }
        }
      }
    }
    phase(P0{}, T1{}, tile);
    phase(P1{}, T1{}, tile);
    phase(P2{}, T1{}, tile);
    phase(P3{}, T1{}, tile);
  }
  if (wr == 0) __builtin_amdgcn_s_barrier();
  __builtin_amdgcn_sched_barrier(0);

  float* sc = (float*)(smem + w * G4_SCR);
  const bool nts = p.nt_store != 0;
#pragma unroll
  for (int mh = 0; mh < 2; ++mh)
#pragma unroll
    for (int mt = 0; mt < 4; ++mt) {
#pragma unroll
      for (int nh = 0; nh < 2; ++nh)
#pragma unroll
        for (int nt = 0; nt < 2; ++nt) *(f32x4*)(sc + r16 * G4_SCR_LD + nh * 32 + nt * 16 + 4 * g) = acc[mh][mt][nh][nt];
      __builtin_amdgcn_wave_barrier();
#pragma unroll
      for (int pass = 0; pass < 2; ++pass) {
        const int r = pass * 8 + (lane >> 3), c = (lane & 7) * 8;
        const int64_t grow = m0 + wr * 128 + mh * 64 + mt * 16 + r;
        const int gcol = n0 + wc * 64 + c;
        if (grow < M && gcol < N) {
          float v[8];
          const f32x4 t0 = *(const f32x4*)(sc + r * G4_SCR_LD + c), t1 = *(const f32x4*)(sc + r * G4_SCR_LD + c + 4);
          if constexpr (SK) {
            float* pd = p.partials + ((size_t)split * (size_t)M + (size_t)grow) * (size_t)N + gcol;
            *(f32x4*)pd = t0, *(f32x4*)(pd + 4) = t1;
            continue;
          }
#pragma unroll
          for (int j = 0; j < 4; ++j) v[j] = t0[j] * p.alpha, v[4 + j] = t1[j] * p.alpha;
          bf16_t* dst = p.C + grow * p.ldc + gcol;
          if (p.beta != 0.f) {
            const u32x4 old = *(const u32x4*)dst;
            const G4_T* o = (const G4_T*)&old;
#pragma unroll
            for (int j = 0; j < 8; ++j) v[j] += p.beta * (float)o[j];
          }
          if (p.bias) {
            const u32x4 bv = *(const u32x4*)(p.bias + gcol);
            const G4_T* b = (const G4_T*)&bv;
#pragma unroll
            for (int j = 0; j < 8; ++j) v[j] += (float)b[j];
          }
          u32x4 pk;
#pragma unroll
          for (int j = 0; j < 4; ++j) pk[j] = G4_PACK(v[2 * j], v[2 * j + 1]);
          if (nts) asm volatile("global_store_dwordx4 %0, %1, off nt\n\ts_nop 1" ::"v"(dst), "v"(pk) : "memory");
          else *(u32x4*)dst = pk;
        }
      }
      __builtin_amdgcn_wave_barrier();
    }
  if constexpr (HF) {
    if (n0 == 0 && p.Hout) {
#pragma unroll
      for (int it = 0; it < 4; ++it) {
        const int idx = it * G4_THREADS + t;
        const int half = idx >> 10, lr = (idx >> 3) & 127, pc = idx & 7;
        const int q = pc ^ ((lr >> 1) & 7);
        const int64_t grow = m0 + (lr >> 6) * 128 + half * 64 + (lr & 63);
        if (grow < M) {
          u32x4 v = *(const u32x4*)(smem + G4_HIMG + half * G4_HALF + lr * 128 + pc * 16);
          if (q == 7 && p.r < 64) v[3] = (v[3] & 0xffffu) | (G4_ONE << 16);
          *(u32x4*)(p.Hout + grow * 64 + q * 8) = v;
        }
      }
    }
  }
}

__global__ __launch_bounds__(256) void G4_REDUCE(const float* __restrict__ part, int splits, int64_t M, int N,
                                                                  G4_T* C, int64_t ldc, const G4_T* bias, float alpha, float beta) {
  const int64_t idx = (int64_t)blockIdx.x * 256 + threadIdx.x;
  const int n8 = N / 8;
  if (idx >= M * n8) return;
  const int64_t row = idx / n8;
  const int col = (int)(idx % n8) * 8;
  const float* src = part + row * N + col;
  f32x4 a0 = __builtin_nontemporal_load((const f32x4*)src), a1 = __builtin_nontemporal_load((const f32x4*)(src + 4));
  for (int s = 1; s < splits; ++s) {
    const float* q = src + (size_t)s * (size_t)M * (size_t)N;
    a0 += __builtin_nontemporal_load((const f32x4*)q), a1 += __builtin_nontemporal_load((const f32x4*)(q + 4));
  }
  float v[8] = {a0[0] * alpha, a0[1] * alpha, a0[2] * alpha, a0[3] * alpha, a1[0] * alpha, a1[1] * alpha, a1[2] * alpha, a1[3] * alpha};
  G4_T* dst = C + row * ldc + col;
  if (beta != 0.f) {
    const u32x4 old = *(const u32x4*)dst;
    const G4_T* o = (const G4_T*)&old;
#pragma unroll
    for (int j = 0; j < 8; ++j) v[j] += beta * (float)o[j];
  }
  if (bias) {
    const u32x4 bv = *(const u32x4*)(bias + col);
    const G4_T* b = (const G4_T*)&bv;
#pragma unroll
    for (int j = 0; j < 8; ++j) v[j] += (float)b[j];
  }
  u32x4 pk;
#pragma unroll
  for (int j = 0; j < 4; ++j) pk[j] = G4_PACK(v[2 * j], v[2 * j + 1]);
  *(u32x4*)dst = pk;
}
```

sow_amd/csrc/kernels.hpp:

```cpp
#pragma once
#include "common.hpp"

namespace sow {
struct ChainParams {
  const void* X;
  void* Y;
  const void *F1a, *F1b, *F2a, *F2b;
  void* Hsave;
  const void* bias;
  int64_t M, ldx, ldy, ldf1a, ldf1b, ldf2a, ldf2b;
  int D1, D2, ra, rb;
  float scale, beta;
  int fast_factors;
  const void* pad_src;
  void* pad_dst;
  int pad_rows, pad_r;
  int ntb, st_per, sl_per;
  float* Hpartial;
  const void* Hload;
  int nt_store;
  int nt_load;
  int pair_flush;
  void* planes;
  size_t planes_bytes;
};
int launch_chain(ChainParams p, int dtype, bool bwd, hipStream_t stream);
constexpr int C2_MAXG = 4;
struct ChainGroup {
  ChainParams p[C2_MAXG];
  int start[C2_MAXG + 1];
  int n;
  uint64_t* stamps;
};
extern void* g_chain2_stamps;
bool chain2_supported(const ChainParams& p, int dtype);
int launch_chain2(const ChainParams& p, bool bwd, int dtype, hipStream_t stream);
int launch_chain2_group(const ChainParams* ps, int n, bool bwd, int dtype, hipStream_t stream);
bool chain2_shared_supported(const ChainParams* ps, int n, bool bwd, int dtype);
int launch_chain2_shared(const ChainParams* ps, int n, bool bwd, int dtype, hipStream_t stream);
int launch_h_reduce(const float* Hpartial, int nsplit, void* Hsave, int64_t M, int rb, float scale, int dtype,
                    hipStream_t stream);
bool chain2f_supported(const ChainParams& p, int dtype);
int launch_chain2f(const ChainParams& p, bool bwd, hipStream_t stream);
size_t chain3f_plane_bytes(int d_in, int d_out);
bool chain3f_supported(const ChainParams& p, int dtype);
int launch_chain3f(const ChainParams& p, bool bwd, hipStream_t stream);
struct TnJob {
  const void* M;
  const void* S;
  float* partial;
  int64_t ldm;
  int D;
  int ones_col;
  int ncg;
  int vec;
  int ones_col_in_s;
};
struct TnParams {
  TnJob job[2];
  int njobs;
  int64_t T;
  int ns;
  int slab_len;
};
struct ReduceJob {
  const float* partial;
  void* out;
  void* colsum;
  int64_t out_ld;
  int D, Dpad, r;
  int transpose;
  int ones_col;
  float alpha, beta;
  int ns;
};
struct ReduceParams {
  ReduceJob job[2];
  int njobs;
  int ns;
  int blocks0;
};
int tn_pick_slabs(int64_t T, int total_colgroups, int total_colgroup_pairs, int total_colgroup_quads, int dtype, int* slab_len);
bool tn_f32q_shape_ok(int64_t T, int d_in, int d_out);
size_t tn_partial_bytes(int ns, int D);
bool tn_f32q_ok(const TnParams& p);
int launch_tn_f32q(const TnParams& p, hipStream_t stream);
int launch_tn(const TnParams& p, int dtype, hipStream_t stream);
constexpr int TN_MAXG = 8;
struct TnGroup {
  TnParams p[TN_MAXG];
  int start[TN_MAXG + 1];
  int n;
};
bool tn_group_supported(const TnParams& p, int dtype);
struct TnRowsItem {
  const void* M;
  const void* S;
  float* partial;
  int64_t ldm, T;
  int D, ncg;
  int nr, gpr, cgw;
  int ns, slab_len;
  int start;
};
constexpr int TNR_MAXI = 2 * TN_MAXG;
struct TnRowsGroup {
  TnRowsItem it[TNR_MAXI];
  int n, total;
  int nt_load;
};
constexpr int TNR_MAX_SLABS = 40;
bool tn_rows_plan(const int64_t* T, const int* D, const int* cap, int n, int* ns_out, int* slab_len_out);
int launch_tn_rows(TnRowsItem* items, int n, hipStream_t stream);
int launch_tn_group(const TnParams* ps, int n, hipStream_t stream);
int launch_tn_reduce(ReduceParams p, int dtype, hipStream_t stream);
int launch_tn_reduce_batch(const ReduceParams* descs, const int* starts, int n, int total_blocks, int dtype, hipStream_t stream);
struct WideArgs {
  const void* X;
  void* Y;
  const void *F1, *F2;
  int64_t ldf1, ldf2;
  void* Hsave;
  const void* bias;
  int64_t M;
  int D1, D2, r;
  float hscale, yscale, beta;
  int bwd;
  void* pack;
  size_t pack_bytes;
};
bool chain_wide_shape_ok(int r, int d1, int d2, int dtype);
bool ragged_shape_ok(int r, int d1, int d2, int dtype);
size_t chain_wide_pack_bytes(int r, int d_in, int d_out);
int launch_chain_wide(const WideArgs& a, int dtype, hipStream_t stream);
struct TnwParams {
  const void* M[2];
  const void* S[2];
  float* partial[2];
  float* colsum;
  int D[2], ncg[2];
  int64_t T;
  int r, r_pad, ns, slab_len;
};
struct TnwReduce {
  const float *P0, *P1, *CS;
  void *dA, *dB, *dbias;
  int D0, D1, r, r_pad, ns;
  float scale, beta;
};
bool tnw_shape_ok(int r, int d_in, int d_out, int dtype);
int tnw_pick_slabs(int64_t T, int d_in, int d_out, int* slab_len);
size_t tnw_partial_bytes(int64_t T, int d_in, int d_out, int r);
int launch_tn_wide(const void* x, const void* dh, const void* dy, const void* h, void* dA, void* dB, void* dbias, int64_t T,
                   int d_in, int d_out, int r, float scale, float beta, int dtype, int out_dtype, void* ws, size_t ws_bytes,
                   hipStream_t stream);
constexpr int SK_MAXL = 16;
struct SkLayer {
  const void *x, *W, *A, *B, *bias;
  void* y;
  float *Py, *Ph;
  int T, d_in, d_out, r;
  int S, KS, ncr, startA, startB;
  float scale;
};
void skinny_plan(int d_in, int d_out, int acc_kind, int* S, int* KS, int* ncr);
size_t skinny_py_bytes(int64_t T, int d_out, int S);
size_t skinny_ph_bytes(int64_t T, int S);
int launch_skinny_fwd(const SkLayer* layers, int n, int dtype, hipStream_t stream);
int launch_gemm(const void* A, int64_t lda, bool transA, const void* B, int64_t ldb, bool transB, void* C, int64_t ldc,
                const void* bias, int64_t M, int N, int K, float alpha, float beta, int dtype, hipStream_t stream);
int launch_gemm_out(const void* A, int64_t lda, bool transA, const void* B, int64_t ldb, bool transB, void* C, int64_t ldc,
                    const void* bias, int64_t M, int N, int K, float alpha, float beta, int dtype, int c_dtype,
                    hipStream_t stream);
bool gemm_rag_supported(const void* A, int64_t lda, const void* B, int64_t ldb, bool transB, const void* C, int64_t ldc, int64_t M,
                        int N, int K, int dtype);
int launch_gemm_rag(const void* A, int64_t lda, const void* B, int64_t ldb, bool transB, void* C, int64_t ldc, int64_t M, int N,
                    int K, int dtype, hipStream_t stream);
int launch_gemm_x3(const void* A, int64_t lda, bool transA, const void* B, int64_t ldb, bool transB, void* C, int64_t ldc,
                   const void* bias, int64_t M, int N, int K, float alpha, float beta, hipStream_t stream);
bool gemm2_supported(const void* A, int64_t lda, const void* B, int64_t ldb, bool nt, const void* A2, int64_t lda2,
                     const void* B2, int64_t ldb2, const void* C, int64_t ldc, const void* bias, int64_t M, int N, int K,
                     int dtype);
int launch_gemm2(const void* A, int64_t lda, const void* B, int64_t ldb, bool nt, const void* A2, int64_t lda2,
                 const void* B2, int64_t ldb2, int k2, void* C, int64_t ldc, const void* bias, int64_t M, int N, int K,
                 float alpha, float beta, hipStream_t stream, void* ws = nullptr, size_t ws_bytes = 0);
int launch_pad64(const void* in, void* out, int rows, int r, hipStream_t stream);
int launch_gemm3(const void* A, int64_t lda, const void* B, int64_t ldb, bool nt, const void* A2, int64_t lda2,
                 const void* B2, int64_t ldb2, int k2, void* C, int64_t ldc, const void* bias, int64_t M, int N, int K,
                 float alpha, float beta, hipStream_t stream);
bool gemm4_supported(const void* A, int64_t lda, const void* B, int64_t ldb, bool nt, const void* A2, int64_t lda2,
                     const void* B2, int64_t ldb2, const void* C, int64_t ldc, const void* bias, int64_t M, int N, int K,
                     int dtype);
int launch_gemm4(const void* A, int64_t lda, const void* B, int64_t ldb, bool nt, const void* A2, int64_t lda2,
                 const void* B2, int64_t ldb2, int k2, void* C, int64_t ldc, const void* bias, int64_t M, int N, int K,
                 float alpha, float beta, hipStream_t stream, void* ws = nullptr, size_t ws_bytes = 0, int dtype = SOW_BF16);
size_t gemm4_splitk_bytes(int64_t M, int N, int K, bool has_ext);
int gemm4_splits(int64_t M, int N, int K, bool has_ext, const void* ws, size_t ws_bytes);
bool gemm4h_supported(const void* X, int64_t ldx, const void* W, int64_t ldw, bool nt, const void* F, int64_t ldf,
                      const void* G, int64_t ldg, const void* C, int64_t ldc, const void* bias, const void* H, int64_t M,
                      int N, int K, int r, int dtype);
int launch_gemm4h(const void* X, int64_t ldx, const void* W, int64_t ldw, bool nt, const void* F, int64_t ldf,
                  const void* G, int64_t ldg, void* C, int64_t ldc, const void* bias, void* H, int64_t M, int N, int K,
                  int r, float hscale, int dtype, hipStream_t stream);
bool gemm2h_supported(const void* X, int64_t ldx, const void* W, int64_t ldw, bool nt, const void* F, int64_t ldf,
                      const void* G, int64_t ldg, const void* C, int64_t ldc, const void* bias, const void* H, int64_t M,
                      int N, int K, int r, int dtype);
int launch_gemm2h(const void* X, int64_t ldx, const void* W, int64_t ldw, bool nt, const void* F, int64_t ldf,
                  const void* G, int64_t ldg, void* C, int64_t ldc, const void* bias, void* H, int64_t M, int N, int K,
                  int r, float hscale, hipStream_t stream);
struct Gemm2hArgs {
  const void *X, *W, *F, *G;
  void* C;
  const void* bias;
  void* H;
  int64_t M, ldx, ldw, ldf, ldg, ldc;
  int N, K, r;
  float hscale;
};
int launch_gemm2h_group(const Gemm2hArgs* a, int n, bool nt, hipStream_t stream);
int launch_gemm3s(const void* A, int64_t lda, const void* B, int64_t ldb, bool nt, const void* A2, int64_t lda2,
                  const void* B2, int64_t ldb2, int k2, void* C, int64_t ldc, const void* bias, int64_t M, int N, int K,
                  float alpha, float beta, hipStream_t stream);
int launch_cast_copy(const void* src, int64_t lds, int src_dtype, void* dst, int64_t ldd, int dst_dtype, int64_t rows,
                     int cols, hipStream_t stream);
int launch_qr_panel(const void* W, int64_t ldw, int in_dtype, int m, int kc, int r, float* Pt, float* Qt,
                    hipStream_t stream);
int launch_qr_copy_out(const float* Qt, const float* Pt, void* Q, int64_t ldq, void* R, int64_t ldr, int out_dtype, int m,
                       int kc, int r, int k_rows, hipStream_t stream);
size_t qr_blocked_t_floats(int kc);
int launch_qr_blocked(const void* W, int64_t ldw, int in_dtype, int m, int kc, int r, float* Pt, float* Qt, float* T,
                      hipStream_t stream);
struct QrItem {
  float* Pt;
  float* Qt;
  int m, kc, r_new, pad;
};
int launch_qr_panel_batch(const QrItem* items, int n, hipStream_t stream);
struct AccItem {
  void* acc;
  const void* A;
  const void* B;
  const void* draw;
  void* A_new;
  float* Pt;
  float* Qt;
  int64_t ld_draw;
  int d_in, d_out, r, r_new, kc;
  float scale, beta;
};
constexpr int ACC_MAXB = 40;
struct AccBatch {
  AccItem it[ACC_MAXB];
  int n;
};
static_assert(sizeof(AccBatch) <= 4096, "by-value kernel arguments must stay under 4 KiB");
int launch_accumulate_batch(const AccItem* items, int n, int dtype, hipStream_t stream);
int launch_multi_zero(void* const* ptrs, const int64_t* bytes, int n, hipStream_t stream);
int launch_adamw_flat(void* p, const void* g, void* m, void* v, int64_t n, float lr, double b1, double b2, float eps,
                      float wd, int step, float grad_scale, int dtype, int state_dtype, hipStream_t stream);
int launch_ttadam_dense(float* p, const float* g, float* m, float* v, int64_t n, double b1, double b2, float eps,
                        float step_size, float lr_wd, int clamp_v, hipStream_t stream);
int launch_tt_kron_core(const float* A, const float* B, float* out, int ra0, int rb0, int ij, int ra1, int rb1,
                        hipStream_t stream);
int launch_absmax(const float* x, int64_t n, float* out, hipStream_t stream);
int launch_small_inverse(const float* A, float* out, int batch, int r, hipStream_t stream);
int launch_axpby(const void* x, void* y, int64_t n, float a, float b, int dtype, hipStream_t stream);
struct PackItem {
  const float* src;
  void* dst;
  int64_t n;
};
int launch_pack_params(const PackItem* items, int n, int dtype, hipStream_t stream);
}
```

Before: 8.680 million.

## Batch gemm4 layer launches into a persistent grouped kernel across layers

Adds grouped variants of the gemm4 and gemm4h kernels. A persistent grid of up to 256 blocks walks a concatenated tile space covering up to four layers, with layers sorted by K. The forward and backward-data group paths now collect fused-H gemm4 calls and eligible plain gemm4 layers, which take an H-only chain2 pass followed by a grouped gemm4, and flush them in batches rather than launching per layer. The intent is to cut per-layer launch overhead and tail underutilisation in the 56-layer stack. In exchange it adds code complexity, more register state (lane-derived indices are recomputed after barriers), and possible ordering or eligibility changes, including a relaxed tile threshold when GEMM4 is forced.

```diff
diff --git a/sow_amd/csrc/api.hip b/sow_amd/csrc/api.hip
--- a/sow_amd/csrc/api.hip
+++ b/sow_amd/csrc/api.hip
@@ -48,7 +48,7 @@
                                                    "NO_GEMM3S",      "GEMM3S",         "GEMM3",      "NO_GROUPED",     "NO_PERSIST",     "NO_NT_STORE",    "NT_LOAD",        "NO_PAIR_FLUSH",  "F32_EXACT",
                                                    "NO_PARK16",      "TN_NO_NT_LOAD",  "NO_TN_ROWS",     "GEMM4",          "NO_GEMM4H",      "NO_CHAIN3F",     "NO_TN_F32Q",     "NO_SPLITK",
                                                    "NO_WIDE_CHAIN",  "NO_SHARED_X",    "NO_RAGGED",      "NO_RAGGED_GEMM", "NO_BLOCKED_QR",
-                                                   "NO_SKINNY"};
+                                                   "NO_SKINNY",      "NO_GROUPED_GEMM4", "GEMM4_GROUP_GRID3"};
 static std::atomic<int> g_switch[SW_COUNT];
 static std::once_flag g_switch_once;
 static void switches_from_env() {
@@ -143,7 +143,7 @@
 
 extern "C" {
 
-int sow_version(void) { return 118; }
+int sow_version(void) { return 119; }
 
 int sow_set_switch(const char* name, int value) {
   if (!name) return SOW_ERR_NULL;
@@ -827,15 +827,73 @@
   return launch_pack_params(items.data(), (int)items.size(), cd, (hipStream_t)stream);
 }
 
+static bool grouped_gemm4_on() { return !sw_on(SW_NO_GROUPED_GEMM4) && !sw_on(SW_NO_GROUPED); }
+
+static bool group_gemm4_plain(const sow_layer_args& L, bool bwd, int dtype, void* dh, void* apad, ChainParams* hp, Gemm4Args* ga) {
+  if (dtype != SOW_BF16 || L.acc_kind != SOW_ACC_DENSE || L.r_live > 64 || !grouped_gemm4_on()) return false;
+  const int N = bwd ? L.d_in : L.d_out, K = bwd ? L.d_out : L.d_in;
+  if (ceil_div(L.T, 64) <= SHORT_NTB && (K + 63) / 64 >= 24) return false;
+  const int64_t tiles = (int64_t)ceil_div(L.T, 256) * ceil_div(N, 256);
+  const int g4 = sw(SW_GEMM4);
+  if (!(g4 > 0 || (g4 < 0 && tiles >= 120)) || K < 64 || gemm4_splitk_bytes(L.T, N, K, true) != 0) return false;
+  ChainParams p{};
+  Gemm4Args a{};
+  if (!bwd) {
+    if (!L.h_save) return false;
+    if (gemm4h_supported(L.x, L.d_in, L.acc_down, L.d_out, false, L.A, L.r_live, L.B, L.d_out, L.y, L.d_out, L.bias, L.h_save, L.T,
+                         L.d_out, L.d_in, L.r_live, dtype) ||
+        gemm2h_supported(L.x, L.d_in, L.acc_down, L.d_out, false, L.A, L.r_live, L.B, L.d_out, L.y, L.d_out, L.bias, L.h_save, L.T,
+                         L.d_out, L.d_in, L.r_live, dtype))
+      return false;
+    p.X = L.x, p.Y = nullptr, p.Hsave = L.h_save, p.bias = nullptr;
+    p.M = L.T, p.ldx = L.d_in, p.ldy = L.d_out, p.D1 = L.d_in, p.D2 = 0;
+    p.F1b = L.A, p.ldf1b = L.r_live, p.F2b = L.B, p.ldf2b = L.d_out, p.rb = L.r_live;
+    a = Gemm4Args{L.x, L.acc_down, L.h_save, L.B, L.y, L.bias, L.T, L.d_in, L.d_out, 64, L.d_out, L.d_out, L.d_out, L.d_in, L.r_live,
+                  1.f, 0.f};
+  } else {
+    if (gemm4h_supported(L.dy, L.d_out, L.acc_down, L.d_out, true, L.B, L.d_out, L.A, L.r_live, L.dx, L.d_in, nullptr, dh, L.T, L.d_in,
+                         L.d_out, L.r_live, dtype) ||
+        gemm2h_supported(L.dy, L.d_out, L.acc_down, L.d_out, true, L.B, L.d_out, L.A, L.r_live, L.dx, L.d_in, nullptr, dh, L.T, L.d_in,
+                         L.d_out, L.r_live, dtype))
+      return false;
+    if ((int64_t)ceil_div(L.T, 64) * 64 < L.d_in) return false;
+    p.X = L.dy, p.Y = nullptr, p.Hsave = dh, p.bias = nullptr;
+    p.M = L.T, p.ldx = L.d_out, p.ldy = L.d_in, p.D1 = L.d_out, p.D2 = 0;
+    p.F1b = L.B, p.ldf1b = L.d_out, p.F2b = L.A, p.ldf2b = L.r_live, p.rb = L.r_live;
+    p.pad_src = L.A, p.pad_dst = apad, p.pad_rows = L.d_in, p.pad_r = L.r_live;
+    a = Gemm4Args{L.dy, L.acc_down, dh, apad, L.dx, nullptr, L.T, L.d_out, L.d_out, 64, 64, L.d_in, L.d_in, L.d_out, 64, 1.f, 0.f};
+  }
+  p.scale = L.scale, p.beta = 0.f;
+  if (!chain2_supported(p, dtype)) return false;
+  const void* Bp = bwd ? p.F1b : p.F2b;
+  const int64_t ldB = bwd ? p.ldf1b : p.ldf2b;
+  const void* Ap = bwd ? p.F2b : p.F1b;
+  if ((reinterpret_cast<uintptr_t>(Bp) & 15) || ldB % 8 || (reinterpret_cast<uintptr_t>(Ap) & 3)) return false;
+  if (!gemm2_supported(a.A, a.lda, a.B, a.ldb, bwd, a.A2, a.lda2, a.B2, a.ldb2, a.C, a.ldc, a.bias, a.M, a.N, a.K, dtype) ||
+      !gemm4_supported(a.A, a.lda, a.B, a.ldb, bwd, a.A2, a.lda2, a.B2, a.ldb2, a.C, a.ldc, a.bias, a.M, a.N, a.K, dtype))
+    return false;
+  *hp = p, *ga = a;
+  return true;
+}
+static int flush_gemm4_plain(const ChainParams* hb, const Gemm4Args* gb, int n, bool bwd, int dtype, hipStream_t stream) {
+  if (n <= 0) return SOW_OK;
+  const int rc = launch_chain2_group(hb, n, bwd, dtype, stream);
+  return rc ? rc : launch_gemm4_group(gb, n, bwd, dtype, stream);
+}
+
 static int forward_group_impl(const sow_layer_args* layers, int n, int dtype, void* stream_) {
   hipStream_t stream = (hipStream_t)stream_;
   if (!ok_dtype(dtype)) return SOW_ERR_DTYPE;
   if (n < 0) return SOW_ERR_SHAPE;
   if (n == 0) return SOW_OK;
   if (!layers) return SOW_ERR_NULL;
-  ChainParams batch[C2_MAXG];
+  ChainParams batch[C2_MAXG], hbatch[G4_MAXG];
   Gemm2hArgs gbatch[4];
-  int nb = 0, ng = 0, rc;
+  Gemm4hArgs g4h[G4_MAXG];
+  Gemm4Args g4p[G4_MAXG];
+  static_assert(G4_MAXG <= C2_MAXG, "the H-only launches of a plain gemm4 batch go out as one chain2 group");
+  int nb = 0, ng = 0, n4h = 0, n4p = 0, rc;
+  const bool grp4 = grouped_gemm4_on();
   for (int i = 0; i < n; ++i) {
     const sow_layer_args& L = layers[i];
     if ((rc = check_layer(L, false))) return rc;
@@ -851,9 +909,19 @@
     if (L.acc_kind == SOW_ACC_DENSE && L.r_live <= 64 && L.h_save &&
         gemm4h_supported(L.x, L.d_in, L.acc_down, L.d_out, false, L.A, L.r_live, L.B, L.d_out, L.y, L.d_out, L.bias, L.h_save, L.T,
                          L.d_out, L.d_in, L.r_live, dtype)) {
-      if ((rc = launch_gemm4h(L.x, L.d_in, L.acc_down, L.d_out, false, L.A, L.r_live, L.B, L.d_out, L.y, L.d_out, L.bias, L.h_save,
-                              L.T, L.d_out, L.d_in, L.r_live, L.scale, dtype, stream)))
-        return rc;
+      g4h[n4h++] = Gemm4hArgs{L.x, L.acc_down, L.A, L.B, L.y, L.bias, L.h_save, L.T, L.d_in, L.d_out, L.r_live, L.d_out, L.d_out,
+                              L.d_out, L.d_in, L.r_live, L.scale};
+      if (n4h == G4_MAXG || !grp4) {
+        if ((rc = launch_gemm4h_group(g4h, n4h, false, dtype, stream))) return rc;
+        n4h = 0;
+      }
+      continue;
+    }
+    if (group_gemm4_plain(L, false, dtype, nullptr, nullptr, &hbatch[n4p], &g4p[n4p])) {
+      if (++n4p == G4_MAXG) {
+        if ((rc = flush_gemm4_plain(hbatch, g4p, n4p, false, dtype, stream))) return rc;
+        n4p = 0;
+      }
       continue;
     }
     if (L.acc_kind == SOW_ACC_DENSE && L.r_live <= 64 && L.h_save && !sw_on(SW_NO_GROUPED) &&
@@ -872,6 +940,8 @@
     if (rc) return rc;
   }
   if (ng && (rc = launch_gemm2h_group(gbatch, ng, false, stream))) return rc;
+  if (n4h && (rc = launch_gemm4h_group(g4h, n4h, false, dtype, stream))) return rc;
+  if ((rc = flush_gemm4_plain(hbatch, g4p, n4p, false, dtype, stream))) return rc;
   return nb ? launch_chain2_group(batch, nb, false, dtype, stream) : SOW_OK;
 }
 
@@ -962,9 +1032,12 @@
     return plan_ws(L.T, L.d_in, L.d_out, L.r_live, L.acc_kind == SOW_ACC_LOWRANK ? L.r_acc : 0, L.acc_kind, dtype);
   };
   if (do_data) {
-    ChainParams batch[C2_MAXG];
+    ChainParams batch[C2_MAXG], hbatch[G4_MAXG];
     Gemm2hArgs gbatch[4];
-    int nb = 0, ng = 0;
+    Gemm4hArgs g4h[G4_MAXG];
+    Gemm4Args g4p[G4_MAXG];
+    int nb = 0, ng = 0, n4h = 0, n4p = 0;
+    const bool grp4 = grouped_gemm4_on();
     for (int i = 0; i < n; ++i) {
       const sow_layer_args& L = layers[i];
       if (L.T == 0) {
@@ -982,9 +1055,12 @@
       } else if (L.acc_kind == SOW_ACC_DENSE && L.r_live <= 64 &&
                  gemm4h_supported(L.dy, L.d_out, L.acc_down, L.d_out, true, L.B, L.d_out, L.A, L.r_live, L.dx, L.d_in, nullptr, dh,
                                   L.T, L.d_in, L.d_out, L.r_live, dtype)) {
-        if ((rc = launch_gemm4h(L.dy, L.d_out, L.acc_down, L.d_out, true, L.B, L.d_out, L.A, L.r_live, L.dx, L.d_in, nullptr, dh,
-                                L.T, L.d_in, L.d_out, L.r_live, L.scale, dtype, stream)))
-          return rc;
+        g4h[n4h++] = Gemm4hArgs{L.dy, L.acc_down, L.B, L.A, L.dx, nullptr, dh, L.T, L.d_out, L.d_out, L.d_out, L.r_live, L.d_in,
+                                L.d_in, L.d_out, L.r_live, L.scale};
+        if (n4h == G4_MAXG || !grp4) {
+          if ((rc = launch_gemm4h_group(g4h, n4h, true, dtype, stream))) return rc;
+          n4h = 0;
+        }
       } else if (L.acc_kind == SOW_ACC_DENSE && L.r_live <= 64 && !sw_on(SW_NO_GROUPED) &&
                  gemm2h_supported(L.dy, L.d_out, L.acc_down, L.d_out, true, L.B, L.d_out, L.A, L.r_live, L.dx, L.d_in, nullptr, dh,
                                   L.T, L.d_in, L.d_out, L.r_live, dtype)) {
@@ -994,10 +1070,17 @@
           if ((rc = launch_gemm2h_group(gbatch, ng, true, stream))) return rc;
           ng = 0;
         }
+      } else if (group_gemm4_plain(L, true, dtype, dh, ws_base(L.workspace) + w.off_apad, &hbatch[n4p], &g4p[n4p])) {
+        if (++n4p == G4_MAXG) {
+          if ((rc = flush_gemm4_plain(hbatch, g4p, n4p, true, dtype, stream))) return rc;
+          n4p = 0;
+        }
       } else if ((rc = single(L, SOW_BWD_DATA)))
         return rc;
     }
     if (ng && (rc = launch_gemm2h_group(gbatch, ng, true, stream))) return rc;
+    if (n4h && (rc = launch_gemm4h_group(g4h, n4h, true, dtype, stream))) return rc;
+    if ((rc = flush_gemm4_plain(hbatch, g4p, n4p, true, dtype, stream))) return rc;
     if (nb && (rc = launch_chain2_group(batch, nb, true, dtype, stream))) return rc;
   }
   int rns[TNR_MAXI], rslab[TNR_MAXI];
diff --git a/sow_amd/csrc/common.hpp b/sow_amd/csrc/common.hpp
--- a/sow_amd/csrc/common.hpp
+++ b/sow_amd/csrc/common.hpp
@@ -150,6 +150,8 @@
   SW_NO_RAGGED_GEMM,
   SW_NO_BLOCKED_QR,
   SW_NO_SKINNY,
+  SW_NO_GROUPED_GEMM4,
+  SW_GEMM4_GROUP_GRID3,
   SW_COUNT
 };
 int sw(int which);
diff --git a/sow_amd/csrc/gemm4.hip b/sow_amd/csrc/gemm4.hip
--- a/sow_amd/csrc/gemm4.hip
+++ b/sow_amd/csrc/gemm4.hip
@@ -37,6 +37,13 @@
   float* partials;
 };
 
+struct Gemm4Group {
+  Gemm4Params p[G4_MAXG];
+  int start[G4_MAXG + 1];
+  int n;
+};
+static_assert(sizeof(Gemm4Group) <= 4096, "by-value kernel arguments must stay under 4 KiB");
+
 __device__ __forceinline__ f32x4 mfma16(u32x4 a, u32x4 b, f32x4 c) {
   return __builtin_amdgcn_mfma_f32_16x16x32_bf16(as_bf16x8(a), as_bf16x8(b), c, 0, 0, 0);
 }
@@ -77,12 +84,20 @@
   g4_rdtr<NH * G4_HALF + 8192 + 1024>(bh[1][1], n1a);
 }
 
+__device__ __forceinline__ int g4_lane_id() {
+  int l;
+  asm volatile("v_mbcnt_lo_u32_b32 %0, -1, 0\n\tv_mbcnt_hi_u32_b32 %0, -1, %0" : "=v"(l));
+  return l;
+}
+
 enum : int { G4_A0 = 0, G4_B0 = 1, G4_B1 = 2, G4_A1 = 3 };
 template <int KIND> __device__ __forceinline__ constexpr int g4_slot_off() {
   return KIND == G4_A0 ? G4_OFF_A0 : KIND == G4_A1 ? G4_OFF_A1 : KIND == G4_B0 ? G4_OFF_B0 : G4_OFF_B1;
 }
 
 #define G4_KERNEL gemm4_kernel
+#define G4_TILE gemm4_tile
+#define G4_GROUP gemm4_group_kernel
 #define G4_REDUCE gemm4_splitk_reduce_kernel
 #define G4_T bf16_t
 #define G4_MFMA mfma16
@@ -90,12 +105,16 @@
 #define G4_ONE 0x3F80u
 #include "gemm4_body.hpp"
 #undef G4_KERNEL
+#undef G4_TILE
+#undef G4_GROUP
 #undef G4_REDUCE
 #undef G4_T
 #undef G4_MFMA
 #undef G4_PACK
 #undef G4_ONE
 #define G4_KERNEL gemm4_f16_kernel
+#define G4_TILE gemm4_f16_tile
+#define G4_GROUP gemm4_f16_group_kernel
 #define G4_REDUCE gemm4_f16_splitk_reduce_kernel
 #define G4_T f16_t
 #define G4_MFMA mfma16_f16
@@ -103,6 +122,8 @@
 #define G4_ONE 0x3C00u
 #include "gemm4_body.hpp"
 #undef G4_KERNEL
+#undef G4_TILE
+#undef G4_GROUP
 #undef G4_REDUCE
 #undef G4_T
 #undef G4_MFMA
@@ -147,11 +168,9 @@
   return (s > 1 && ws && ws_bytes >= gemm4_splitk_bytes(M, N, K, has_ext)) ? s : 1;
 }
 
-int launch_gemm4(const void* A, int64_t lda, const void* B, int64_t ldb, bool nt, const void* A2, int64_t lda2,
-                 const void* B2, int64_t ldb2, int k2, void* C, int64_t ldc, const void* bias, int64_t M, int N, int K,
-                 float alpha, float beta, hipStream_t stream, void* ws, size_t ws_bytes, int dtype) {
-  if (dtype != SOW_BF16 && dtype != SOW_F16) return SOW_ERR_DTYPE;
-  const bool f16 = dtype == SOW_F16;
+static Gemm4Params g4_params(const void* A, int64_t lda, const void* B, int64_t ldb, const void* A2, int64_t lda2, const void* B2,
+                             int64_t ldb2, int k2, void* C, int64_t ldc, const void* bias, int64_t M, int N, int K, float alpha,
+                             float beta) {
   Gemm4Params p;
   p.A = (const bf16_t*)A, p.B = (const bf16_t*)B, p.A2 = (const bf16_t*)A2, p.B2 = (const bf16_t*)B2;
   p.C = (bf16_t*)C, p.bias = (const bf16_t*)bias;
@@ -162,6 +181,15 @@
   p.nt_store = SOW_GEMM_NT(M) ? 1 : 0;
   p.F = nullptr, p.ldf = 0, p.Hout = nullptr, p.r = 0, p.hscale = 0.f;
   p.splits = 1, p.kt_per = 0, p.partials = nullptr;
+  return p;
+}
+
+int launch_gemm4(const void* A, int64_t lda, const void* B, int64_t ldb, bool nt, const void* A2, int64_t lda2,
+                 const void* B2, int64_t ldb2, int k2, void* C, int64_t ldc, const void* bias, int64_t M, int N, int K,
+                 float alpha, float beta, hipStream_t stream, void* ws, size_t ws_bytes, int dtype) {
+  if (dtype != SOW_BF16 && dtype != SOW_F16) return SOW_ERR_DTYPE;
+  const bool f16 = dtype == SOW_F16;
+  Gemm4Params p = g4_params(A, lda, B, ldb, A2, lda2, B2, ldb2, k2, C, ldc, bias, M, N, K, alpha, beta);
   const int64_t tiles = (int64_t)ceil_div(M, G4_BM) * ceil_div(N, G4_BN);
   if (tiles <= 0) return SOW_OK;
   if (tiles > 0x7fffffff) return SOW_ERR_SHAPE;
@@ -211,7 +239,7 @@
   if (sw_on(SW_NO_FUSED_H) || sw_on(SW_FORCE_GEMM_V1) || sw(SW_GEMM4) == 0 || sw_on(SW_NO_GEMM4H)) return false;
   if (r < 2 || r > 64 || (r & 1) || N < 64 || K < 64) return false;
   const int tiles_n = ceil_div(N, G4_BN);
-  if (tiles_n > 2 || (int64_t)ceil_div(M, G4_BM) * tiles_n < 120) return false;
+  if (tiles_n > 2 || (sw(SW_GEMM4) <= 0 && (int64_t)ceil_div(M, G4_BM) * tiles_n < 120)) return false;
   if (K % 8 || N % 8 || ldx % 8 || ldw % 8 || ldc % 8) return false;
   if (!g4_al16(X) || !g4_al16(W) || !g4_al16(C) || !g4_al16(H) || (bias && !g4_al16(bias))) return false;
   auto al4 = [](const void* q) { return (reinterpret_cast<uintptr_t>(q) & 3) == 0; };
@@ -223,11 +251,9 @@
   return true;
 }
 
-int launch_gemm4h(const void* X, int64_t ldx, const void* W, int64_t ldw, bool nt, const void* F, int64_t ldf,
-                  const void* G, int64_t ldg, void* C, int64_t ldc, const void* bias, void* H, int64_t M, int N, int K,
-                  int r, float hscale, int dtype, hipStream_t stream) {
-  if (dtype != SOW_BF16 && dtype != SOW_F16) return SOW_ERR_DTYPE;
-  const bool f16 = dtype == SOW_F16;
+static Gemm4Params g4h_params(const void* X, int64_t ldx, const void* W, int64_t ldw, bool nt, const void* F, int64_t ldf, const void* G,
+                              int64_t ldg, void* C, int64_t ldc, const void* bias, void* H, int64_t M, int N, int K, int r,
+                              float hscale) {
   Gemm4Params p;
   p.A = (const bf16_t*)X, p.B = (const bf16_t*)W, p.A2 = nullptr, p.B2 = (const bf16_t*)G;
   p.C = (bf16_t*)C, p.bias = (const bf16_t*)bias;
@@ -238,6 +264,15 @@
   p.nt_store = SOW_GEMM_NT(M) ? 1 : 0;
   p.F = (const bf16_t*)F, p.ldf = ldf, p.Hout = (bf16_t*)H, p.r = r, p.hscale = hscale;
   p.splits = 1, p.kt_per = 0, p.partials = nullptr;
+  return p;
+}
+
+int launch_gemm4h(const void* X, int64_t ldx, const void* W, int64_t ldw, bool nt, const void* F, int64_t ldf,
+                  const void* G, int64_t ldg, void* C, int64_t ldc, const void* bias, void* H, int64_t M, int N, int K,
+                  int r, float hscale, int dtype, hipStream_t stream) {
+  if (dtype != SOW_BF16 && dtype != SOW_F16) return SOW_ERR_DTYPE;
+  const bool f16 = dtype == SOW_F16;
+  Gemm4Params p = g4h_params(X, ldx, W, ldw, nt, F, ldf, G, ldg, C, ldc, bias, H, M, N, K, r, hscale);
   const int64_t tiles = (int64_t)ceil_div(M, G4_BM) * ceil_div(N, G4_BN);
   if (tiles <= 0) return SOW_OK;
   if (tiles > 0x7fffffff) return SOW_ERR_SHAPE;
@@ -254,4 +289,92 @@
   return SOW_OK;
 }
 
-}
+constexpr int G4_RESIDENT = 256;
+static int g4_launch_group(Gemm4Params* ps, int n, bool nt, bool hf, int dtype, hipStream_t stream) {
+  Gemm4Group g{};
+  int order[G4_MAXG];
+  for (int i = 0; i < n; ++i) order[i] = i;
+  for (int i = 1; i < n; ++i)
+    for (int j = i; j > 0 && ps[order[j]].K > ps[order[j - 1]].K; --j) {
+      const int tmp = order[j];
+      order[j] = order[j - 1], order[j - 1] = tmp;
+    }
+  int64_t total = 0;
+  int m = 0;
+  for (int i = 0; i < n; ++i) {
+    const Gemm4Params& p = ps[order[i]];
+    const int64_t tiles = (int64_t)ceil_div(p.M, G4_BM) * ceil_div(p.N, G4_BN);
+    if (tiles <= 0) continue;
+    g.p[m] = p;
+    g.start[m++] = (int)total;
+    total += tiles;
+    if (total > 0x7fffffff) return SOW_ERR_SHAPE;
+  }
+  g.n = m;
+  for (int i = m; i <= G4_MAXG; ++i) g.start[i] = (int)total;
+  if (total <= 0) return SOW_OK;
+  const int cap = sw_on(SW_GEMM4_GROUP_GRID3) ? 3 : G4_RESIDENT;
+  const int64_t grid = total < cap ? total : cap;
+  const bool f16 = dtype == SOW_F16;
+#define G4G_LAUNCH(K, LDS, ...)                                                                                  \
+  do {                                                                                                           \
+    SOW_SET_MAX_LDS_ONCE(LDS, K<__VA_ARGS__>);                                                                   \
+    hipLaunchKernelGGL((K<__VA_ARGS__>), dim3((unsigned)grid), dim3(G4_THREADS), LDS, stream, g);               \
+  } while (0)
+  if (hf && nt) {
+    if (f16) G4G_LAUNCH(gemm4_f16_group_kernel, G4_LDS_H, true, true);
+    else G4G_LAUNCH(gemm4_group_kernel, G4_LDS_H, true, true);
+  } else if (hf) {
+    if (f16) G4G_LAUNCH(gemm4_f16_group_kernel, G4_LDS_H, false, true);
+    else G4G_LAUNCH(gemm4_group_kernel, G4_LDS_H, false, true);
+  } else if (nt) {
+    if (f16) G4G_LAUNCH(gemm4_f16_group_kernel, G4_LDS, true, false);
+    else G4G_LAUNCH(gemm4_group_kernel, G4_LDS, true, false);
+  } else {
+    if (f16) G4G_LAUNCH(gemm4_f16_group_kernel, G4_LDS, false, false);
+    else G4G_LAUNCH(gemm4_group_kernel, G4_LDS, false, false);
+  }
+#undef G4G_LAUNCH
+  SOW_CHECK_LAUNCH();
+  return SOW_OK;
+}
+
+int launch_gemm4h_group(const Gemm4hArgs* a, int n, bool nt, int dtype, hipStream_t stream) {
+  if (n <= 0) return SOW_OK;
+  if (dtype != SOW_BF16 && dtype != SOW_F16) return SOW_ERR_DTYPE;
+  if (n > G4_MAXG) return SOW_ERR_SHAPE;
+  if (n == 1 || sw_on(SW_NO_GROUPED_GEMM4)) {
+    for (int i = 0; i < n; ++i) {
+      const int rc = launch_gemm4h(a[i].X, a[i].ldx, a[i].W, a[i].ldw, nt, a[i].F, a[i].ldf, a[i].G, a[i].ldg, a[i].C, a[i].ldc, a[i].bias,
+                                   a[i].H, a[i].M, a[i].N, a[i].K, a[i].r, a[i].hscale, dtype, stream);
+      if (rc) return rc;
+    }
+    return SOW_OK;
+  }
+  Gemm4Params ps[G4_MAXG];
+  for (int i = 0; i < n; ++i)
+    ps[i] = g4h_params(a[i].X, a[i].ldx, a[i].W, a[i].ldw, nt, a[i].F, a[i].ldf, a[i].G, a[i].ldg, a[i].C, a[i].ldc, a[i].bias, a[i].H,
+                       a[i].M, a[i].N, a[i].K, a[i].r, a[i].hscale);
+  return g4_launch_group(ps, n, nt, true, dtype, stream);
+}
+
+int launch_gemm4_group(const Gemm4Args* a, int n, bool nt, int dtype, hipStream_t stream) {
+  if (n <= 0) return SOW_OK;
+  if (dtype != SOW_BF16 && dtype != SOW_F16) return SOW_ERR_DTYPE;
+  if (n > G4_MAXG) return SOW_ERR_SHAPE;
+  if (n == 1 || sw_on(SW_NO_GROUPED_GEMM4)) {
+    for (int i = 0; i < n; ++i) {
+      const int rc = launch_gemm4(a[i].A, a[i].lda, a[i].B, a[i].ldb, nt, a[i].A2, a[i].lda2, a[i].B2, a[i].ldb2, a[i].k2, a[i].C, a[i].ldc,
+                                  a[i].bias, a[i].M, a[i].N, a[i].K, a[i].alpha, a[i].beta, stream, nullptr, 0, dtype);
+      if (rc) return rc;
+    }
+    return SOW_OK;
+  }
+  Gemm4Params ps[G4_MAXG];
+  for (int i = 0; i < n; ++i)
+    ps[i] = g4_params(a[i].A, a[i].lda, a[i].B, a[i].ldb, a[i].A2, a[i].lda2, a[i].B2, a[i].ldb2, a[i].k2, a[i].C, a[i].ldc, a[i].bias,
+                      a[i].M, a[i].N, a[i].K, a[i].alpha, a[i].beta);
+  return g4_launch_group(ps, n, nt, false, dtype, stream);
+}
+
+}
diff --git a/sow_amd/csrc/gemm4_body.hpp b/sow_amd/csrc/gemm4_body.hpp
--- a/sow_amd/csrc/gemm4_body.hpp
+++ b/sow_amd/csrc/gemm4_body.hpp
@@ -1,15 +1,13 @@
 
-template <bool NT, bool HF, bool SK = false> __global__ __launch_bounds__(G4_THREADS, 2) void G4_KERNEL(const Gemm4Params p) {
-  extern __shared__ __attribute__((aligned(16))) char smem[];
-  const int t = threadIdx.x, lane = t & 63;
+
+template <bool NT, bool HF, bool SK, bool GRP> __device__ __forceinline__ void G4_TILE(const Gemm4Params& p, char* smem, const int t,
+                                                                                    const int lid, const int split) {
+  int lane = t & 63;
   const int w = __builtin_amdgcn_readfirstlane(t >> 6);
   const int wr = w >> 2, wc = w & 3;
-  const int r16 = lane & 15, g = lane >> 4;
+  int r16 = lane & 15, g = lane >> 4;
   const int tiles_n = (p.N + G4_BN - 1) / G4_BN;
   const int splits = SK ? p.splits : 1;
-  const int ntiles = (int)gridDim.x / splits;
-  const int split = splits > 1 ? (int)blockIdx.x / ntiles : 0;
-  const int lid = splits > 1 ? (int)blockIdx.x % ntiles : xcd_remap(blockIdx.x, gridDim.x);
   const int64_t m0 = (int64_t)(lid / tiles_n) * G4_BM;
   const int n0 = (lid % tiles_n) * G4_BN;
   const int K = p.K, N = p.N;
@@ -22,7 +20,7 @@
   const int H = 4 * NTL;
   const char* zp = zero_page_for(lane);
 
-  const int c_pc = lane & 7;
+  int c_pc = lane & 7;
   int c_lr[2], c_q[2];
 #pragma unroll
   for (int ii = 0; ii < 2; ++ii) {
@@ -37,15 +35,32 @@
     const int gn = n0 + (lr >> 5) * 64 + nh * 32 + (lr & 31);
     return gn < N ? gn : N - 1;
   };
-  const int m_kr0 = 8 * w + (lane >> 4);
-  const int m_f = (((lane >> 4) & 3) | ((w & 1) << 2)) << 1;
-  const int m_q = (lane & 15) ^ m_f;
+  int m_kr0 = 8 * w + (lane >> 4);
+  int m_f = (((lane >> 4) & 3) | ((w & 1) << 2)) << 1;
+  int m_q = (lane & 15) ^ m_f;
   auto b_col_nn = [&](int nh) -> int {
     const int lc = 8 * m_q;
     const int gn = n0 + (lc >> 5) * 64 + nh * 32 + (lc & 31);
     return gn + 8 <= N ? gn : N - 8;
   };
 
+  auto reseed = [&]() {
+    if constexpr (GRP) {
+      lane = g4_lane_id();
+      r16 = lane & 15, g = lane >> 4;
+      zp = zero_page_for(lane);
+      c_pc = lane & 7;
+#pragma unroll
+      for (int ii = 0; ii < 2; ++ii) {
+        c_lr[ii] = 16 * w + 8 * ii + (lane >> 3);
+        c_q[ii] = c_pc ^ ((c_lr[ii] >> 1) & 7);
+      }
+      m_kr0 = 8 * w + (lane >> 4);
+      m_f = (((lane >> 4) & 3) | ((w & 1) << 2)) << 1;
+      m_q = (lane & 15) ^ m_f;
+    }
+  };
+
   const bf16_t* pA[2][2];
   const bf16_t* pB[2][2];
 #pragma unroll
@@ -53,6 +68,7 @@
 #pragma unroll
     for (int ii = 0; ii < 2; ++ii) {
       pA[hh][ii] = p.A + a_row(hh, c_lr[ii]) * p.lda + 8 * c_q[ii];
+      if constexpr (HF) continue;
       if constexpr (NT) pB[hh][ii] = p.B + (int64_t)b_col_nt(hh, c_lr[ii]) * p.ldb + 8 * c_q[ii];
       else pB[hh][ii] = p.B + (int64_t)(m_kr0 + 4 * ii) * p.ldb + b_col_nn(hh);
     }
@@ -218,6 +234,7 @@
         for (int mt = 0; mt < 4; ++mt) hacc[1][mt] = G4_MFMA(ffr[ks], xa[mt][ks], hacc[1][mt]);
       __builtin_amdgcn_sched_barrier(0);
     }
+    reseed();
 #pragma unroll
     for (int mh = 0; mh < 2; ++mh)
 #pragma unroll
@@ -236,7 +253,11 @@
 #pragma unroll
     for (int hh = 0; hh < 2; ++hh)
 #pragma unroll
-      for (int ii = 0; ii < 2; ++ii) pA[hh][ii] = p.A + a_row(hh, c_lr[ii]) * p.lda + 8 * c_q[ii];
+      for (int ii = 0; ii < 2; ++ii) {
+        pA[hh][ii] = p.A + a_row(hh, c_lr[ii]) * p.lda + 8 * c_q[ii];
+        if constexpr (NT) pB[hh][ii] = p.B + (int64_t)b_col_nt(hh, c_lr[ii]) * p.ldb + 8 * c_q[ii];
+        else pB[hh][ii] = p.B + (int64_t)(m_kr0 + 4 * ii) * p.ldb + b_col_nn(hh);
+      }
   }
 
   const uint32_t base = lds_addr(smem);
@@ -404,6 +425,8 @@
   if (wr == 0) __builtin_amdgcn_s_barrier();
   __builtin_amdgcn_sched_barrier(0);
 
+  reseed();
+  const int tq = GRP ? 64 * w + lane : t;
   float* sc = (float*)(smem + w * G4_SCR);
   const bool nts = p.nt_store != 0;
 #pragma unroll
@@ -456,7 +479,7 @@
     if (n0 == 0 && p.Hout) {
 #pragma unroll
       for (int it = 0; it < 4; ++it) {
-        const int idx = it * G4_THREADS + t;
+        const int idx = it * G4_THREADS + tq;
         const int half = idx >> 10, lr = (idx >> 3) & 127, pc = idx & 7;
         const int q = pc ^ ((lr >> 1) & 7);
         const int64_t grow = m0 + (lr >> 6) * 128 + half * 64 + (lr & 63);
@@ -467,6 +490,36 @@
         }
       }
     }
+  }
+}
+
+template <bool NT, bool HF, bool SK = false> __global__ __launch_bounds__(G4_THREADS, 2) void G4_KERNEL(const Gemm4Params p) {
+  extern __shared__ __attribute__((aligned(16))) char smem[];
+  const int splits = SK ? p.splits : 1;
+  const int ntiles = (int)gridDim.x / splits;
+  const int split = splits > 1 ? (int)blockIdx.x / ntiles : 0;
+  const int lid = splits > 1 ? (int)blockIdx.x % ntiles : xcd_remap(blockIdx.x, gridDim.x);
+  G4_TILE<NT, HF, SK, false>(p, smem, (int)threadIdx.x, lid, split);
+}
+
+template <bool NT, bool HF> __global__ __launch_bounds__(G4_THREADS, 2) void G4_GROUP(const Gemm4Group grp) {
+  extern __shared__ __attribute__((aligned(16))) char smem[];
+  const int w = __builtin_amdgcn_readfirstlane((int)threadIdx.x >> 6);
+  const int total = grp.start[G4_MAXG];
+  const int grid = (int)gridDim.x;
+  for (int base = 0; base < total; base += grid) {
+    const int nr = total - base < grid ? total - base : grid;
+    if ((int)blockIdx.x >= nr) break;
+    const int v = base + xcd_remap(blockIdx.x, nr);
+    int layer = 0;
+#pragma unroll
+    for (int i = 1; i < G4_MAXG; ++i)
+      if (i < grp.n && v >= grp.start[i]) layer = i;
+    const int tt = 64 * w + g4_lane_id();
+    G4_TILE<NT, HF, false, true>(grp.p[layer], smem, tt, v - grp.start[layer], 0);
+    asm volatile("s_waitcnt lgkmcnt(0)" ::: "memory");
+    __builtin_amdgcn_s_barrier();
+    __builtin_amdgcn_sched_barrier(0);
   }
 }
 
diff --git a/sow_amd/csrc/kernels.hpp b/sow_amd/csrc/kernels.hpp
--- a/sow_amd/csrc/kernels.hpp
+++ b/sow_amd/csrc/kernels.hpp
@@ -202,6 +202,26 @@
 int launch_gemm4h(const void* X, int64_t ldx, const void* W, int64_t ldw, bool nt, const void* F, int64_t ldf,
                   const void* G, int64_t ldg, void* C, int64_t ldc, const void* bias, void* H, int64_t M, int N, int K,
                   int r, float hscale, int dtype, hipStream_t stream);
+constexpr int G4_MAXG = 4;
+struct Gemm4hArgs {
+  const void *X, *W, *F, *G;
+  void* C;
+  const void* bias;
+  void* H;
+  int64_t M, ldx, ldw, ldf, ldg, ldc;
+  int N, K, r;
+  float hscale;
+};
+int launch_gemm4h_group(const Gemm4hArgs* a, int n, bool nt, int dtype, hipStream_t stream);
+struct Gemm4Args {
+  const void *A, *B, *A2, *B2;
+  void* C;
+  const void* bias;
+  int64_t M, lda, ldb, lda2, ldb2, ldc;
+  int N, K, k2;
+  float alpha, beta;
+};
+int launch_gemm4_group(const Gemm4Args* a, int n, bool nt, int dtype, hipStream_t stream);
 bool gemm2h_supported(const void* X, int64_t ldx, const void* W, int64_t ldw, bool nt, const void* F, int64_t ldf,
                       const void* G, int64_t ldg, const void* C, int64_t ldc, const void* bias, const void* H, int64_t M,
                       int N, int K, int r, int dtype);
```

After: 8.625 million. About the same (-0.6%).
